# sjy-dv/coltt

Hardware: AMD Instinct MI355X
Metric: queries/sec @ recall@10, 10Mx768 HNSW (higher is better)
Workload: dtype f32

## Files before the change

### coltt_amd/_lib.py

```python
import ctypes as C
import os
import re

HERE = os.path.dirname(os.path.abspath(__file__))
COSINE, EUCLIDEAN = 0, 1
Q_NONE, Q_F16, Q_F8, Q_BF16 = 0, 1, 2, 3
SELECT_REFERENCE, SELECT_NEAREST = 0, 1
MODE_EXACT, MODE_MFMA = 0, 1
NBR_NONE = 0xFFFFFFFF

_lib = None
_env_seen = None
_KNOBS = ("COLTT_FLAT_ONE", "COLTT_FLAT_IDS_CHUNK", "COLTT_STAGING", "COLTT_EV8", "COLTT_ROWS8", "COLTT_F8_MFMA", "COLTT_VISG", "COLTT_WALK2", "COLTT_WALK2_LDS", "COLTT_BLOOM_KB",
          "COLTT_WAVES_PER_CU", "COLTT_ROWS_NT", "COLTT_ROWS_NT_MIN_MB", "COLTT_ROW_FILTER", "COLTT_ROW_FILTER_BITS", "COLTT_ROW_FILTER_UPPER", "COLTT_DESCENT_NT", "COLTT_ROW_SHADOW", "COLTT_ROW_SHADOW_BITS", "COLTT_VIS16", "COLTT_VIS16_BUCKET_BITS", "COLTT_PQ_WAVES", "COLTT_PQ_NBR", "COLTT_PQ_NBR_PATCH", "COLTT_LAT_SEQ", "COLTT_LAT_HELPERS", "COLTT_LAT_MAX_NQ", "COLTT_MW_MAX_NQ", "COLTT_VISG_BUDGET_MB")


class ColttError(RuntimeError):
    def __init__(self, code, msg):
        super().__init__(f"coltt_gpu error {code}: {msg}")
        self.code = code


def lib_path():
    return os.environ.get("COLTT_LIB", os.path.join(HERE, "libcoltt_gpu.so"))


def declared_symbols():
    hdr = open(os.path.join(HERE, "..", "include", "coltt_gpu.h")).read()
    return sorted(set(re.findall(r"\b(coltt_[a-z0-9_]+)\s*\(", hdr)))


def _sync_policy():
    global _env_seen
    get = os.environ.get
    now = tuple(get(k) for k in _KNOBS)
    if now != _env_seen:
        if _env_seen is not None:
            _lib.coltt_policy_reload()
        _env_seen = now


def lib():
    global _lib
    if _lib is not None:
        _sync_policy()
        return _lib
    if _lib is None:
        try:
            import torch
        except Exception:
            pass
        p = lib_path()
        if not os.path.exists(p):
            raise ColttError(-5, f"{p} is missing — build it with `python -m coltt_amd.build` "
                                 "(hipcc --offload-arch=gfx950); there is no CPU fallback")
        L = C.CDLL(p)
        L.coltt_last_error.restype = C.c_char_p
        L.coltt_version.restype = C.c_char_p
        if hasattr(L, "coltt_hnsw_pq_search_filtered_batch"):
            L.coltt_hnsw_pq_search_filtered_batch.restype = C.c_int
            L.coltt_hnsw_pq_search_filtered_batch.argtypes = [C.c_uint64, C.c_void_p, C.c_void_p, C.c_size_t, C.c_uint32, C.c_uint32, C.c_uint32, C.c_int,
                                                              C.c_void_p, C.c_void_p, C.c_void_p, C.c_void_p, C.c_void_p]
        if hasattr(L, "coltt_flat_mfma_eligible_host"):
            L.coltt_flat_mfma_eligible_host.restype = C.c_int
            L.coltt_flat_mfma_eligible_host.argtypes = [C.c_int, C.c_int, C.c_uint32, C.c_float, C.c_float, C.c_int]
        _lib = L
        _sync_policy()
    return _lib


def check(rc):
    if rc != 0:
        raise ColttError(rc, lib().coltt_last_error().decode("utf-8", "replace"))


def vp(a):
    if a is None:
        return C.c_void_p(0)
    if isinstance(a, int):
        return C.c_void_p(a)
    return a.ctypes.data_as(C.c_void_p)
```

### coltt_amd/csrc/common.hip

```cpp
#include "common.hpp"

#include <algorithm>
#include <cstdlib>

namespace coltt {

thread_local std::string g_last_error;
static int g_device = -1;
static std::mutex g_dev_mu;

Registry& Registry::get() {
  static Registry r;
  return r;
}
coltt_handle_t Registry::add(std::shared_ptr<Object> o) {
  std::lock_guard<std::mutex> g(mu_);
  coltt_handle_t h = next_++;
  map_[h] = std::move(o);
  return h;
}
std::shared_ptr<Object> Registry::find(coltt_handle_t h) {
  std::lock_guard<std::mutex> g(mu_);
  auto it = map_.find(h);
  return it == map_.end() ? nullptr : it->second;
}
bool Registry::erase(coltt_handle_t h) {
  std::shared_ptr<Object> keep;
  {
    std::lock_guard<std::mutex> g(mu_);
    auto it = map_.find(h);
    if (it == map_.end()) return false;
    keep = it->second;
    map_.erase(it);
  }
  WriteLock g2(keep->rw);
  return true;
}

int ensure_device() {
  int dev;
  {
    std::lock_guard<std::mutex> g(g_dev_mu);
    if (g_device < 0) {
      int n = 0;
      hipError_t e = hipGetDeviceCount(&n);
      if (e != hipSuccess || n <= 0)
        return fail(COLTT_E_DEVICE, "libcoltt_gpu: no HIP device visible (%s) — this library has no CPU fallback",
                    e == hipSuccess ? "device count 0" : hipGetErrorString(e));
      g_device = 0;
    }
    dev = g_device;
  }
  COLTT_HIP(hipSetDevice(dev));
  return COLTT_OK;
}

int default_device() { std::lock_guard<std::mutex> g(g_dev_mu); return g_device < 0 ? 0 : g_device; }

int use_device(int device) {
  COLTT_HIP(hipSetDevice(device));
  return COLTT_OK;
}

namespace {
std::shared_mutex g_pol_mu;
Policy g_policy;
bool g_policy_loaded = false;
Policy read_policy_from_env() {
  Policy p;
  auto off = [](const char* n) { const char* e = getenv(n); return e && *e == '0'; };
  auto num = [](const char* n, bool& set) -> long long { const char* e = getenv(n); set = e && *e; return set ? atoll(e) : 0; };
  bool set = false; long long v;
  p.flat_one = !off("COLTT_FLAT_ONE"); p.staging = !off("COLTT_STAGING"); p.ev8 = !off("COLTT_EV8"); { const char* e = getenv("COLTT_ROWS8"); p.rows8 = (!e || !*e) ? 1 : (*e == '0' ? 0 : (*e == '2' ? 2 : 1)); } p.f8_mfma = !off("COLTT_F8_MFMA");
  v = num("COLTT_FLAT_IDS_CHUNK", set); p.flat_ids_chunk = set && v > 0 ? (uint32_t)((std::min<long long>(v, 1ll << 30) + 31) / 32 * 32) : 0u;
  v = num("COLTT_VISG", set); p.visg = set ? (int)v : -1;
  { const char* e = getenv("COLTT_WALK2"); p.walk2 = (!e || !*e) ? 7 : (!strcmp(e, "off") ? -1 : (atoi(e) & 15)); }
  { const char* e = getenv("COLTT_WALK2_LDS"); if (!e || !*e) p.walk2_lds = 4; else if (!strcmp(e, "off")) p.walk2_lds = -1; else { const int w = atoi(e) & 6; p.walk2_lds = w ? w : -1; } }
  v = num("COLTT_BLOOM_KB", set); p.bloom_kb = set ? (int)std::max<long long>(1, std::min<long long>(64, v)) : 0;
  v = num("COLTT_WAVES_PER_CU", set); p.waves_per_cu = set ? (int)std::max<long long>(1, std::min<long long>(12, v)) : 0;
  v = num("COLTT_ROWS_NT", set); p.rows_nt = set ? (v > 0 ? 1 : (v < 0 ? -1 : 0)) : -1;
  v = num("COLTT_ROW_FILTER", set); p.row_filter = set ? (v > 0 ? 1 : 0) : -1;
  v = num("COLTT_ROW_FILTER_UPPER", set); p.row_filter_upper = set ? (v > 0 ? 1 : 0) : -1;
  v = num("COLTT_DESCENT_NT", set); p.descent_nt = set ? (v > 0 ? 1 : 0) : -1;
  p.row_shadow = !off("COLTT_ROW_SHADOW");
  v = num("COLTT_ROW_FILTER_BITS", set); p.row_filter_bits = set && (v == 8 || v == 16) ? (int)v : 0;
  { const char* e = getenv("COLTT_ROW_FILTER_BITS"); if (e && !strcmp(e, "8i")) p.row_filter_bits = 80; }
  { const char* e = getenv("COLTT_ROW_SHADOW_BITS"); p.row_shadow_bits = (!e || !*e) ? 8 : (!strcmp(e, "both") ? 24 : (atoi(e) == 16 ? 16 : 8)); }
  v = num("COLTT_ROWS_NT_MIN_MB", set); p.rows_nt_min_mb = set ? std::max<long long>(0, v) : 12288;
  p.vis16 = !off("COLTT_VIS16");
  v = num("COLTT_VIS16_BUCKET_BITS", set); p.vis16_bucket_bits = set ? (int)std::max<long long>(1, std::min<long long>(10, v)) : 0;
  v = num("COLTT_PQ_WAVES", set); p.pq_waves = set ? (int)std::max<long long>(1, std::min<long long>(16, v)) : 0;
  p.pq_nbr = !off("COLTT_PQ_NBR");
  p.pq_nbr_patch = !off("COLTT_PQ_NBR_PATCH");
  { const char* e = getenv("COLTT_LAT_SEQ"); p.lat_seq = e && *e == '1'; }
  v = num("COLTT_LAT_HELPERS", set); p.lat_helpers = set ? (int)std::max<long long>(0, std::min<long long>(3, v)) : 0;
  v = num("COLTT_LAT_MAX_NQ", set); if (!set) v = num("COLTT_MW_MAX_NQ", set);
  p.lat_knob_set = set; p.lat_max_nq = set ? (uint32_t)std::max<long long>(0, v) : 0;
  v = num("COLTT_VISG_BUDGET_MB", set); p.visg_budget_mb = set ? v : -1;
  return p;
}
}

Policy policy() {
  {
    std::shared_lock<std::shared_mutex> g(g_pol_mu);
    if (g_policy_loaded) return g_policy;
  }
  std::unique_lock<std::shared_mutex> g(g_pol_mu);
  if (!g_policy_loaded) { g_policy = read_policy_from_env(); g_policy_loaded = true; }
  return g_policy;
}

size_t max_search_ctx() {
  static const size_t v = [] { const char* e = getenv("COLTT_MAX_SEARCH_CTX"); long n = e && *e ? atol(e) : 32; return (size_t)(n < 1 ? 1 : (n > 256 ? 256 : n)); }();
  return v;
}

}

using namespace coltt;

extern "C" {

int coltt_init(int device) {
  int n = 0;
  hipError_t e = hipGetDeviceCount(&n);
  if (e != hipSuccess || n <= 0)
    return fail(COLTT_E_DEVICE, "coltt_init: no HIP device visible (%s) — this library has no CPU fallback",
                e == hipSuccess ? "device count 0" : hipGetErrorString(e));
  if (device < 0 || device >= n) return fail(COLTT_E_INVALID, "coltt_init: device %d out of range [0,%d)", device, n);
  {
    std::lock_guard<std::mutex> g(g_dev_mu);
    g_device = device;
  }
  COLTT_HIP(hipSetDevice(device));
  return COLTT_OK;
}

int coltt_device_count(void) {
  int n = 0;
  if (hipGetDeviceCount(&n) != hipSuccess) return 0;
  return n;
}

const char* coltt_last_error(void) { return g_last_error.c_str(); }

int coltt_policy_reload(void) {
  Policy p = read_policy_from_env();
  std::unique_lock<std::shared_mutex> g(g_pol_mu);
  g_policy = p; g_policy_loaded = true;
  return COLTT_OK;
}
const char* coltt_version(void) {
  return "coltt_gpu 0.6 (gfx950)";
}

}

#include "exact.hpp"
extern "C" uint64_t coltt_shard_vertex_host(uint64_t id, uint64_t shard_count) {
  return shard_count ? coltt::dev::shard_vertex(id, shard_count) : 0;
}
```

### coltt_amd/csrc/common.hpp

```cpp
#pragma once
#include <hip/hip_runtime.h>

#include <cstdarg>
#include <cstdint>
#include <cstdio>
#include <cstring>
#include <memory>
#include <condition_variable>
#include <mutex>
#include <shared_mutex>
#include <string>
#include <unordered_map>
#include <vector>

#include "../../include/coltt_gpu.h"

namespace coltt {

extern thread_local std::string g_last_error;

inline int fail(int code, const char* fmt, ...) {
  char buf[512];
  va_list ap;
  va_start(ap, fmt);
// ... 7 lines not shown
  do {                                                                                           \
    hipError_t _e = (expr);                                                                      \
    if (_e != hipSuccess)                                                                        \
      return ::coltt::fail(_e == hipErrorOutOfMemory ? COLTT_E_NOMEM : COLTT_E_DEVICE, "%s: %s", \
                           #expr, hipGetErrorString(_e));                                        \
  } while (0)

#define COLTT_TRY(expr)        \
  do {                         \
    int _rc = (expr);          \
    if (_rc != COLTT_OK) return _rc; \
  } while (0)

struct DevBuf {
  void* p = nullptr;
  size_t cap = 0;
  DevBuf() = default;
  DevBuf(const DevBuf&) = delete;
  DevBuf& operator=(const DevBuf&) = delete;
  ~DevBuf() { if (p) (void)hipFree(p); }
  int reserve(size_t bytes, bool keep = false, hipStream_t s = nullptr) {
    if (bytes <= cap) return COLTT_OK;
    size_t ncap = keep ? std::max(bytes, cap + cap / 2) : bytes;
    void* np = nullptr;
    COLTT_HIP(hipMalloc(&np, ncap));
    if (keep && p && cap) {
      hipError_t e = hipMemcpyAsync(np, p, cap, hipMemcpyDeviceToDevice, s);
      if (e == hipSuccess) e = hipStreamSynchronize(s);
      if (e != hipSuccess) {
        (void)hipFree(np);
        return ::coltt::fail(COLTT_E_DEVICE, "DevBuf::reserve copy: %s", hipGetErrorString(e));
      }
    }
    if (p) (void)hipFree(p);
    p = np;
    cap = ncap;
    return COLTT_OK;
  }
  template <class T> T* as() const { return (T*)p; }
};

struct PinnedBuf {
  void* p = nullptr;
  size_t cap = 0;
  PinnedBuf() = default;
  PinnedBuf(const PinnedBuf&) = delete;
  PinnedBuf& operator=(const PinnedBuf&) = delete;
  ~PinnedBuf() { if (p) (void)hipHostFree(p); }
  int reserve(size_t bytes) {
    if (bytes <= cap) return COLTT_OK;
    if (p) { (void)hipHostFree(p); p = nullptr; cap = 0; }
    COLTT_HIP(hipHostMalloc(&p, bytes, hipHostMallocDefault));
    cap = bytes;
    return COLTT_OK;
  }
  template <class T> T* as() const { return (T*)p; }
};
constexpr size_t SMALL_CALL_BYTES = 64 * 1024;

struct Policy {
  bool flat_one = true;
  uint32_t flat_ids_chunk = 0;
  bool staging = true;
  bool ev8 = true;
  bool f8_mfma = true;
  int rows8 = 1;
  int visg = -1;
  int walk2 = 7;
  int walk2_lds = 4;
  int bloom_kb = 0;
  int waves_per_cu = 0;
  int rows_nt = -1;
  int row_filter = -1;
  bool row_shadow = true;
  int row_filter_bits = 0;
  int row_shadow_bits = 8;
  long long rows_nt_min_mb = 12288;
  int row_filter_upper = -1;
  int descent_nt = -1;
  bool vis16 = true;
  int vis16_bucket_bits = 0;
  int pq_waves = 0;
  bool pq_nbr = true;
  bool pq_nbr_patch = true;
  bool lat_seq = false;
  int lat_helpers = 0;
  bool lat_knob_set = false;
  uint32_t lat_max_nq = 0;
  long long visg_budget_mb = -1;
};
Policy policy();
inline bool small_call_staging() { return policy().staging; }

struct Object {
  std::shared_mutex rw;
  int device = 0;
  virtual ~Object() {}
};
typedef std::shared_lock<std::shared_mutex> ReadLock;
typedef std::unique_lock<std::shared_mutex> WriteLock;

size_t max_search_ctx();
template <class C> class CtxPool {
 public:
  C* acquire() {
    std::unique_lock<std::mutex> lk(mu_);
    for (;;) {
      if (!idle_.empty()) { C* c = idle_.back(); idle_.pop_back(); return c; }
      if (all_.size() < max_search_ctx()) {
        auto c = std::make_unique<C>();
        if (c->init() != COLTT_OK) return nullptr;
        C* p = c.get(); all_.push_back(std::move(c)); return p;
      }
      cv_.wait(lk);
    }
  }
  void release(C* c) { { std::lock_guard<std::mutex> lk(mu_); idle_.push_back(c); } cv_.notify_one(); }
  size_t created() { std::lock_guard<std::mutex> lk(mu_); return all_.size(); }
 private:
  std::mutex mu_; std::condition_variable cv_;
  std::vector<std::unique_ptr<C>> all_; std::vector<C*> idle_;
};
template <class C> struct CtxLease {
  CtxPool<C>& pool; C* c;
  explicit CtxLease(CtxPool<C>& p) : pool(p), c(p.acquire()) {}
  ~CtxLease() { if (c) pool.release(c); }
  CtxLease(const CtxLease&) = delete; CtxLease& operator=(const CtxLease&) = delete;
};

class Registry {
 public:
  static Registry& get();
  coltt_handle_t add(std::shared_ptr<Object> o);
  std::shared_ptr<Object> find(coltt_handle_t h);
  bool erase(coltt_handle_t h);

 private:
  std::mutex mu_;
  std::unordered_map<coltt_handle_t, std::shared_ptr<Object>> map_;
  coltt_handle_t next_ = 0x1000;
};

template <class T> std::shared_ptr<T> lookup(coltt_handle_t h) {
  return std::dynamic_pointer_cast<T>(Registry::get().find(h));
}

int ensure_device();
int default_device();
int use_device(int device);

class DeviceScope {
 public:
  DeviceScope() = default;
  DeviceScope(const DeviceScope&) = delete;
  DeviceScope& operator=(const DeviceScope&) = delete;
  ~DeviceScope() { if (prev_ >= 0 && prev_ != cur_) (void)hipSetDevice(prev_); }
  int enter(int device) {
    if (hipGetDevice(&prev_) != hipSuccess) prev_ = -1;
    if (device < 0) { COLTT_TRY(ensure_device()); cur_ = default_device(); return COLTT_OK; }
    COLTT_TRY(use_device(device));
    cur_ = device;
    return COLTT_OK;
  }
  int device() const { return cur_; }
 private:
  int prev_ = -1, cur_ = -1;
// ... 25 lines not shown
```

### coltt_amd/csrc/hnsw.hip

```cpp
#include <algorithm>
#include <atomic>
#include <cmath>
#include <map>

#include "common.hpp"
#include "hnsw_index.hpp"
#include "exact.hpp"
#include "hnsw_dev.hpp"
#include "hnsw_walk2.hpp"
#include "hnsw_lat.hpp"
#include "hnsw_pq.hpp"
#include "prep.hpp"
#include "rows8_ingest.hpp"

#include "hnsw_kernels.hpp"
#include "filter_expr.hpp"
#include "attr_filter.hpp"
#include "hnsw_compact.hpp"

using namespace coltt;
using namespace coltt::dev;
using namespace coltt::kern;
using namespace coltt::hnsw;

// ... 878 lines not shown
  const uint64_t t = (uint64_t)blockIdx.x * blockDim.x + threadIdx.x;
  const uint64_t i = t / per;
  uint32_t n = cap;
  if (count) { const uint32_t c = *count; n = c < cap ? c : cap; }
  if (i >= n) return;
  const uint32_t slot = slots[i];
  if (slot >= n_slots) return;
  const uint32_t r = (uint32_t)(t - i * per);
  const uint32_t p = r / pieces, pc = r - p * pieces;
  const uint64_t e = (uint64_t)slot * W + p;
  const uint32_t nb = adj0[e];
  u32x4v v = {0u, 0u, 0u, 0u};
  if (nb < n_slots) v = *reinterpret_cast<const u32x4v*>(codes + (size_t)nb * row_bytes + (size_t)pc * 16);
  *reinterpret_cast<u32x4v*>(nbr + e * row_bytes + (size_t)pc * 16) = v;
}
constexpr uint64_t PQ_PATCH_MAX_LIST = 1ull << 20;
struct PqNbrPatch { bool on = false; uint32_t* d_dirty = nullptr; uint32_t cap = 0; };
PqNbrPatch pq_nbr_patch_begin(Hnsw* x, uint64_t max_listed) {
  PqNbrPatch t;
  const bool current = !x->pq_nbr_stale.load() && x->pq_nbr_ok;
  x->pq_nbr_stale.store(true);
  if (!current || !x->pq_on || max_listed > PQ_PATCH_MAX_LIST) return t;
  const Policy pol = policy();
  if (!pol.pq_nbr || !pol.pq_nbr_patch) return t;
  if (max_listed) {
    if (x->pq_dirty.reserve((2 + max_listed) * 4) != COLTT_OK) { (void)hipGetLastError(); return t; }
    if (hipMemsetAsync(x->pq_dirty.p, 0, 8, x->stream) != hipSuccess) { (void)hipGetLastError(); return t; }
    t.d_dirty = x->pq_dirty.as<uint32_t>(); t.cap = (uint32_t)max_listed;
  }
  t.on = true;
  return t;
}
int pq_nbr_patch_end(Hnsw* x, const PqNbrPatch& t, uint64_t first_new, uint64_t n_new, const uint32_t* d_slots, uint32_t n_slots_listed) {
  if (!t.on) return COLTT_OK;
  const uint32_t W = (uint32_t)x->cfg.m_max0, pieces = x->pq_row >> 4;
  if (x->pq_nbr.cap < (size_t)std::max<uint64_t>(x->cap, x->n) * W * x->pq_row || x->pq_done < x->n) return COLTT_OK;
  const uint32_t* adj0 = x->adj0.as<uint32_t>(); const uint8_t* codes = x->pq_codes.as<uint8_t>(); uint8_t* nbr = x->pq_nbr.as<uint8_t>();
  if (n_new) {
    const uint64_t total = n_new * W * pieces, e0 = first_new * W;
    pq_nbr_build_kernel<<<(unsigned)ceil_div(total, 256), 256, 0, x->stream>>>(adj0 + e0, codes, nbr + e0 * x->pq_row, total, x->pq_row);
  }
  const uint32_t* list = t.d_dirty ? t.d_dirty + 2 : d_slots;
  const uint32_t lcap = t.d_dirty ? t.cap : n_slots_listed;
  if (lcap) pq_nbr_patch_kernel<<<(unsigned)ceil_div((uint64_t)lcap * W * pieces, 256), 256, 0, x->stream>>>(adj0, codes, nbr, list, t.d_dirty, lcap, W, x->pq_row, (uint32_t)x->n);
  COLTT_HIP(hipGetLastError());
  uint32_t listed = n_slots_listed;
  if (t.d_dirty) COLTT_HIP(hipMemcpyAsync(&listed, t.d_dirty, 4, hipMemcpyDeviceToHost, x->stream));
  COLTT_HIP(hipStreamSynchronize(x->stream));
  if (listed > lcap) return COLTT_OK;
  x->pq_nbr_patches.fetch_add(1); x->pq_nbr_patched_rows.fetch_add(n_new + listed);
  x->pq_nbr_stale.store(false);
  return COLTT_OK;
}
constexpr size_t PQ_WAVES_CAP = 12;
bool pq_geom(Hnsw* x, uint32_t ef, bool force_hbm, PqGeom& out, uint32_t filt_cap = 0) {
  PqGeom s{};
  s.ef = ef; s.ef_pad = (ef + 63) & ~63u;
  const size_t fixed = (size_t)s.ef_pad * 8 + ((size_t)pq_walk_table_rows(x->pq_row >> 4) << pq_lut_shift(x)) * 2
                     + (filt_cap ? (size_t)((filt_cap + 63u) & ~63u) * 8 : 0);
  if (fixed > 160 * 1024) return false;
  const bool hbm_ok = x->vis_stride != 0 && x->vis_regions > 0;
  uint32_t hcap = std::min<uint32_t>(32768u, std::max<uint32_t>(8192u, next_pow2(ef * 48u)));
  const bool lds_fits = fixed + (size_t)hcap * 4 <= 160 * 1024;
  if (!force_hbm && !(wants_visg(policy(), ef) && hbm_ok) && lds_fits) { s.variant = 0; s.vis_words = hcap; s.lds = fixed + (size_t)hcap * 4; }
  else {
    if (!hbm_ok) return false;
    s.variant = 2; s.vis_words = 0; s.lds = fixed;
  }
  {
    const Policy pol = policy();
    const size_t cap = pol.pq_waves > 0 ? (size_t)pol.pq_waves : PQ_WAVES_CAP;
    s.per_cu = (uint32_t)std::max<size_t>(1, std::min<size_t>(cap, (160 * 1024) / s.lds));
  }
  out = s;
  return true;
}

}

namespace coltt {
namespace hnsw {
int launch_pq_walk(Hnsw* x, HCtx* c, const PqGeom& sg, bool nbr, uint32_t grid, uint32_t region_base, const unsigned short* lut, uint32_t nq, uint32_t k,
                   uint32_t rerank, uint32_t* counter, uint32_t* surv, uint32_t* surv_cnt, unsigned long long* stats, const FilterView* fv, uint32_t fcap,
                   const PqFiltQuery* pd) {
  const uint32_t sh = pq_lut_shift(x);
  const uint32_t np = x->pq_row >> 4;
  typedef void (*pq_kern_t)(GraphView, int32_t, int32_t, const unsigned short*, const uint8_t*, const uint8_t*, uint32_t, uint32_t, uint32_t, uint32_t, uint32_t, uint32_t, uint32_t, uint32_t,
                            uint32_t*, uint32_t*, uint32_t*, unsigned long long*, uint8_t*, size_t, uint32_t*, FilterView, uint32_t);
  pq_kern_t kern;
#define COLTT_PQKF(LS, NP, F, P) (sg.variant == 0 ? (pq_kern_t)hnsw_pq_search_kernel<0, VIS_LDS, LS, NP, false, F, P> : nbr ? (pq_kern_t)hnsw_pq_search_kernel<2, VIS_HBM, LS, NP, true, F, P> : (pq_kern_t)hnsw_pq_search_kernel<2, VIS_HBM, LS, NP, false, F, P>)
#define COLTT_PQK(LS, NP) (pd ? COLTT_PQKF(LS, NP, true, true) : fv ? COLTT_PQKF(LS, NP, true, false) : COLTT_PQKF(LS, NP, false, false))
  if (sh == 5 && np == 4) kern = COLTT_PQK(5, 4);
  else if (sh == 4 && np == 4) kern = COLTT_PQK(4, 4);
  else if (sh == 8 && np == 2) kern = COLTT_PQK(8, 2);
  else if (sh == 8 && np == 6) kern = COLTT_PQK(8, 6);
  else if (sh == 4) kern = COLTT_PQK(4, 0);
  else if (sh == 5) kern = COLTT_PQK(5, 0);
  else if (sh == 8) kern = COLTT_PQK(8, 0);
  else kern = COLTT_PQK(0, 0);
#undef COLTT_PQK
#undef COLTT_PQKF
  COLTT_HIP(hipFuncSetAttribute(reinterpret_cast<const void*>(kern), hipFuncAttributeMaxDynamicSharedMemorySize, (int)sg.lds));
  kern<<<grid, 64, sg.lds, c->stream>>>(x->view(), x->entry, x->entry_level, lut, x->pq_codes.as<uint8_t>(), nbr ? x->pq_nbr.as<uint8_t>() : nullptr, x->pq_row, sh, nq, k, sg.ef, sg.ef_pad, rerank,
                                        sg.vis_words, counter, surv, surv_cnt, stats, x->w_visg.as<uint8_t>() + (size_t)region_base * x->vis_stride,
                                        (size_t)x->vis_stride, x->w_vepoch.as<uint32_t>() + region_base,
                                        pd ? FilterView{reinterpret_cast<const uint32_t*>(pd), 0u} : fv ? *fv : FilterView{nullptr, 0u}, fcap);
  COLTT_HIP(hipGetLastError());
  return COLTT_OK;
}
}
}

namespace {
}

namespace coltt {
namespace kern {
__global__ __launch_bounds__(64) void hnsw_pq_select_kernel(const unsigned long long* __restrict__ keys, const uint32_t* __restrict__ surv_cnt, uint32_t ef_pad, uint32_t k,
                                                            const uint64_t* __restrict__ ids, uint64_t* __restrict__ out_ids, float* __restrict__ out_scores,
                                                            uint32_t* __restrict__ out_counts, const PqFiltQuery* __restrict__ pd = nullptr) {
  extern __shared__ __attribute__((aligned(16))) uint8_t smem[];
  unsigned long long* const res = reinterpret_cast<unsigned long long*>(smem);
  const uint32_t qi = blockIdx.x, r = surv_cnt[qi];
  const uint32_t row = pd ? pd[qi].row : qi;
  const int lane_in = threadIdx.x;
  for (uint32_t i = (uint32_t)lane_in; i < r; i += 64) res[i] = keys[(size_t)qi * ef_pad + i];
  wave_sync();
  const uint32_t n = r < k ? r : k;
  for (uint32_t t = 0; t < n; t++) {
    const int lane = opaque_lane(lane_in);
    unsigned long long best = ~0ull; uint32_t bi = 0;
    for (uint32_t i = (uint32_t)lane; i < r; i += 64) { const unsigned long long e = res[i]; if (e < best) { best = e; bi = i; } }
    const unsigned long long km = wave_min_u64(best);
    if (best == km && km != ~0ull) {
      const uint32_t slot = (uint32_t)km >> 1;
      out_ids[(size_t)row * k + t] = ids ? ids[slot] : (uint64_t)slot;
      out_scores[(size_t)row * k + t] = __uint_as_float((uint32_t)(km >> 32));
      res[bi] = ~0ull;
    }
    wave_sync();
  }
  if (lane_in == 0) out_counts[row] = n;
}
}
}

namespace {
template <int METRIC, int QUANT>
int launch_pq_rerank_for(Hnsw* x, HCtx* c, const PqGeom& sg, uint32_t q0, uint32_t nq, uint32_t k, const uint32_t* surv, const uint32_t* surv_cnt,
                     unsigned long long* keys, uint64_t* oi, float* os, uint32_t* oc, const PqFiltQuery* pd = nullptr, const float* pd_qe = nullptr,
                     const float* pd_qn = nullptr) {
  const dim3 grid(ceil_div(sg.ef_pad, 32), nq);
  const GraphView g = x->view();
  const float* qe = c->w_qeff.as<float>() + (size_t)q0 * x->dim; const float* qn = c->w_qn.as<float>() + q0;
  if (pd) { qe = pd_qe; qn = pd_qn; q0 = 0; }
  if (x->r8) hnsw_pq_rerank_kernel<METRIC, QUANT, true><<<grid, 64, 0, c->stream>>>(g, qe, qn, surv, surv_cnt, sg.ef_pad, keys);
  else hnsw_pq_rerank_kernel<METRIC, QUANT, false><<<grid, 64, 0, c->stream>>>(g, qe, qn, surv, surv_cnt, sg.ef_pad, keys);
  const size_t lds = (size_t)sg.ef_pad * 8;
  COLTT_HIP(hipFuncSetAttribute(reinterpret_cast<const void*>(hnsw_pq_select_kernel), hipFuncAttributeMaxDynamicSharedMemorySize, (int)lds));
  hnsw_pq_select_kernel<<<nq, 64, lds, c->stream>>>(keys, surv_cnt, sg.ef_pad, k, g.ids, oi + (size_t)q0 * k, os + (size_t)q0 * k, oc + q0, pd);
  COLTT_HIP(hipGetLastError());
  return COLTT_OK;
}
}

namespace coltt {
namespace hnsw {
int launch_pq_rerank(Hnsw* x, HCtx* c, const PqGeom& sg, uint32_t q0, uint32_t nq, uint32_t k, const uint32_t* surv, const uint32_t* surv_cnt,
                     unsigned long long* keys, uint64_t* oi, float* os, uint32_t* oc, const PqFiltQuery* pd, const float* pd_qe, const float* pd_qn) {
  int rc;
#define COLTT_LP_ARGS x, c, sg, q0, nq, k, surv, surv_cnt, keys, oi, os, oc, pd, pd_qe, pd_qn
#define COLTT_LP(Q) rc = x->metric == COLTT_COSINE ? launch_pq_rerank_for<M_COS, Q>(COLTT_LP_ARGS) : launch_pq_rerank_for<M_L2, Q>(COLTT_LP_ARGS)
  if (x->quant == COLTT_Q_NONE) { COLTT_LP(Q_NONE); } else { COLTT_LP(Q_F16); }
#undef COLTT_LP
#undef COLTT_LP_ARGS
  return rc;
}

int pq_walk_geom(Hnsw* x, uint32_t ef, bool force_hbm, uint32_t fcap, PqGeom& sg) {
  const Policy pol = policy();
  if (wants_visg(pol, ef) || force_hbm) COLTT_TRY(ensure_visg(x, pol));
  bool have = pq_geom(x, ef, force_hbm, sg, fcap);
  if (!have && !force_hbm) { COLTT_TRY(ensure_visg(x, pol)); have = pq_geom(x, ef, true, sg, fcap); }
  if (!have) return fail(COLTT_E_UNSUPPORTED, "hnsw_pq_search: dim %u / ef %u / %u sub-vectors need more than the CU's 160 KiB of LDS", x->dim, ef, x->pq_shape.m);
  return COLTT_OK;
}
}
}

namespace {

int pq_search_once(Hnsw* x, HCtx* c, const float* queries, bool on_device, size_t nq, uint32_t k, uint32_t ef_override, uint32_t rerank,
                   uint64_t* out_ids, float* out_scores, uint32_t* out_counts, coltt_hnsw_stats* stats, uint64_t* out_n_exact, bool force_hbm, bool* retry_hbm,
                   const FilterView* fv = nullptr) {
  *retry_hbm = false;
  if (stats) std::memset(stats, 0, sizeof(*stats));
  if (out_n_exact) *out_n_exact = 0;
  if (nq == 0) return COLTT_OK;
  if (k == 0) return fail(COLTT_E_INVALID, "hnsw_pq_search: k must be >= 1");
  if (!x->pq_on) return fail(COLTT_E_INVALID, "hnsw_pq_search: the index carries no product-quantiser codes (coltt_hnsw_pq_attach)");
  if (x->pq_done != x->n) return fail(COLTT_E_DEVICE, "hnsw_pq_search: codes cover %llu of %llu slots", (unsigned long long)x->pq_done, (unsigned long long)x->n);
  uint64_t* d_oi = out_ids; float* d_os = out_scores; uint32_t* d_oc = out_counts;
  if (!on_device) {
    COLTT_TRY(c->w_out_ids.reserve(nq * k * 8)); COLTT_TRY(c->w_out_sc.reserve(nq * k * 4)); COLTT_TRY(c->w_out_cnt.reserve(nq * 4));
    d_oi = c->w_out_ids.as<uint64_t>(); d_os = c->w_out_sc.as<float>(); d_oc = c->w_out_cnt.as<uint32_t>();
  }
  if (x->entry < 0) {
    COLTT_HIP(hipMemsetAsync(d_oc, 0, nq * 4, c->stream));
    if (!on_device) COLTT_HIP(hipMemcpyAsync(out_counts, d_oc, nq * 4, hipMemcpyDeviceToHost, c->stream));
    COLTT_HIP(hipStreamSynchronize(c->stream));
    return COLTT_OK;
  }
  const uint32_t ef = std::max<uint32_t>(ef_override ? ef_override : (uint32_t)x->cfg.ef, k);
  if (ef > 4096) return fail(COLTT_E_UNSUPPORTED, "hnsw_pq_search: ef=%u > 4096", ef);
  PqGeom sg;
  const uint32_t fcap = fv ? pq_filt_cap(ef, k, rerank) : 0u;
  COLTT_TRY(pq_walk_geom(x, ef, force_hbm, fcap, sg));
  uint32_t grid = (uint32_t)std::min<size_t>(nq, (size_t)256 * sg.per_cu);
  RegionLease lease;
  if (sg.variant != 0) { acquire_regions(x, grid, lease); grid = lease.count; }
  const float* d_q = queries;
  if (!on_device) {
    COLTT_TRY(c->w_qraw.reserve(nq * x->dim * 4));
    COLTT_HIP(hipMemcpyAsync(c->w_qraw.p, queries, nq * x->dim * 4, hipMemcpyHostToDevice, c->stream));
    d_q = c->w_qraw.as<float>();
  }
  COLTT_TRY(prep_queries_any(x, c, d_q, nq));
  bool nbr = false;
  if (sg.variant != 0) COLTT_TRY(ensure_pq_nbr(x, c->stream, &nbr));
  const uint32_t lsh = pq_lut_shift(x);
  const size_t lut_q = ((size_t)x->pq_row << lsh) * 2;
  const size_t group = std::max<size_t>(1, std::min<size_t>({nq, (256ull << 20) / lut_q, (256ull << 20) / ((size_t)sg.ef_pad * 12), (size_t)32768}));
  COLTT_TRY(c->w_pack.reserve(group * lut_q + group * 4));
  COLTT_TRY(c->w_surv.reserve(group * sg.ef_pad * 4)); COLTT_TRY(c->w_scnt.reserve(group * 4)); COLTT_TRY(c->w_keys.reserve(group * sg.ef_pad * 8));
  COLTT_TRY(c->w_misc.reserve(256));
  uint8_t* misc = c->w_misc.as<uint8_t>();
  uint32_t* counter = reinterpret_cast<uint32_t*>(misc);
  unsigned long long* d_stats = reinterpret_cast<unsigned long long*>(misc + 16);
  COLTT_HIP(hipMemsetAsync(misc, 0, 256, c->stream));
  COLTT_HIP(hipEventRecord(c->ev0, c->stream));
  for (size_t q0 = 0; q0 < nq; q0 += group) {
    const size_t gn = std::min(group, nq - q0);
    COLTT_TRY(pq_lut16_batch(c->stream, x->pq_cb.as<float>(), x->pq_shape, c->w_qeff.as<float>() + q0 * x->dim, gn, x->pq_row, lsh,
                             reinterpret_cast<uint32_t*>(c->w_pack.as<uint8_t>() + group * lut_q), c->w_pack.as<unsigned short>()));
    if (q0) COLTT_HIP(hipMemsetAsync(counter, 0, 4, c->stream));
    COLTT_TRY(launch_pq_walk(x, c, sg, nbr, (uint32_t)std::min<size_t>(grid, gn), lease.base, c->w_pack.as<unsigned short>(), (uint32_t)gn, k, rerank, counter, c->w_surv.as<uint32_t>(),
                             c->w_scnt.as<uint32_t>(), d_stats, fv, fcap));
    COLTT_TRY(launch_pq_rerank(x, c, sg, (uint32_t)q0, (uint32_t)gn, k, c->w_surv.as<uint32_t>(), c->w_scnt.as<uint32_t>(), c->w_keys.as<unsigned long long>(), d_oi, d_os, d_oc));
  }
  COLTT_HIP(hipEventRecord(c->ev1, c->stream));
  if (x->dense && x->dense_base) add_base_kernel<<<ceil_div(nq * k, 256), 256, 0, c->stream>>>(d_oi, nq * k, x->dense_base);
  unsigned long long h_stats[5] = {0, 0, 0, 0, 0};
  if (!on_device) {
    COLTT_HIP(hipMemcpyAsync(out_ids, d_oi, nq * k * 8, hipMemcpyDeviceToHost, c->stream));
    COLTT_HIP(hipMemcpyAsync(out_scores, d_os, nq * k * 4, hipMemcpyDeviceToHost, c->stream));
    COLTT_HIP(hipMemcpyAsync(out_counts, d_oc, nq * 4, hipMemcpyDeviceToHost, c->stream));
  }
  COLTT_HIP(hipMemcpyAsync(h_stats, d_stats, 40, hipMemcpyDeviceToHost, c->stream));
#ifdef COLTT_PHASE_TIMING
  unsigned long long h_pt[8] = {0};
  COLTT_HIP(hipMemcpyAsync(h_pt, d_stats + 8, 64, hipMemcpyDeviceToHost, c->stream));
#endif
  COLTT_HIP(hipStreamSynchronize(c->stream));
#ifdef COLTT_PHASE_TIMING
  {
    static const char* nm[8] = {"pop", "adjacency", "visited", "codes+table sum", "admission/evict/flush", "prologue(table, upper levels)", "flush+re-rank+writeout", "-"};
    double tot = 0; for (int i = 0; i < 7; i++) tot += (double)h_pt[i];
    fprintf(stderr, "[phase pq] nq=%zu ef=%u variant=%d per_cu=%u:", nq, sg.ef, sg.variant, sg.per_cu);
    for (int i = 0; i < 7; i++) fprintf(stderr, " %s %.1f%%", nm[i], 100.0 * (double)h_pt[i] / tot);
    fprintf(stderr, "  | ticks/query %.0f, per expansion %.0f\n", tot / (double)nq, tot / (double)std::max<unsigned long long>(1, h_stats[1]));
  }
#endif
  float ms = 0.f;
  (void)hipEventElapsedTime(&ms, c->ev0, c->ev1);
  x->last_ms.store(ms);
  if (sg.variant == 0 && (h_stats[4] & 8ull)) { *retry_hbm = true; return COLTT_OK; }
  if (h_stats[4]) return fail(COLTT_E_DEVICE, "hnsw_pq_search: traversal watchdog tripped (code %llu)", h_stats[4]);
  if (stats) { stats->n_dist = h_stats[0]; stats->n_exp = h_stats[1]; stats->n_hops = h_stats[2]; stats->n_visit_resets = 0; }
  if (out_n_exact) *out_n_exact = h_stats[3];
  return COLTT_OK;
}
int pq_search_common(Hnsw* x, HCtx* c, const float* queries, bool on_device, size_t nq, uint32_t k, uint32_t ef_override, uint32_t rerank,
                     uint64_t* out_ids, float* out_scores, uint32_t* out_counts, coltt_hnsw_stats* stats, uint64_t* out_n_exact) {
  bool retry = false;
  COLTT_TRY(pq_search_once(x, c, queries, on_device, nq, k, ef_override, rerank, out_ids, out_scores, out_counts, stats, out_n_exact, false, &retry));
  if (retry) COLTT_TRY(pq_search_once(x, c, queries, on_device, nq, k, ef_override, rerank, out_ids, out_scores, out_counts, stats, out_n_exact, true, &retry));
  return COLTT_OK;
}
}

namespace coltt {
namespace hnsw {
int pq_search_filtered_walk(Hnsw* x, HCtx* c, const FilterView& fv, const float* queries, size_t nq, uint32_t k, uint32_t ef_walk, uint32_t rerank,
                            uint64_t* out_ids, float* out_scores, uint32_t* out_counts, coltt_hnsw_stats* stats, uint64_t* out_n_exact) {
  bool retry = false;
  COLTT_TRY(pq_search_once(x, c, queries, false, nq, k, ef_walk, rerank, out_ids, out_scores, out_counts, stats, out_n_exact, false, &retry, &fv));
  if (retry) COLTT_TRY(pq_search_once(x, c, queries, false, nq, k, ef_walk, rerank, out_ids, out_scores, out_counts, stats, out_n_exact, true, &retry, &fv));
  return COLTT_OK;
}
}
}

namespace {

__global__ void hnsw_unlink_kernel(GraphView g, const uint32_t* __restrict__ nbs, const int32_t* __restrict__ lvl, uint32_t n) {
  uint32_t t = blockIdx.x * blockDim.x + threadIdx.x;
  if (t >= n) return;
  uint32_t W;
  uint32_t* row = const_cast<uint32_t*>(adj_row(g, nbs[t], lvl[t], W));
  float* drow = lvl[t] == 0 ? g.adj0_d + (size_t)nbs[t] * g.mMax0 : g.adjU_d + ((size_t)g.upper_off[nbs[t]] + (uint32_t)(lvl[t] - 1)) * g.mMax;
  float* nrow = (lvl[t] == 0 && g.adj0_n) ? g.adj0_n + (size_t)nbs[t] * g.mMax0 : nullptr;
  float2* mrow = (lvl[t] == 0 && g.adj0_m) ? g.adj0_m + (size_t)nbs[t] * g.mMax0 : nullptr;
  uint32_t m = 0;
  for (uint32_t i = 0; i < W && row[i] != NBR_NONE; i++) {
    uint32_t sl = row[i]; float dd = drow[i];
    if (!is_deleted(g, sl)) { row[m] = sl; drow[m] = dd; if (nrow) nrow[m] = nrow[i]; if (mrow) mrow[m] = mrow[i]; m++; }
  }
  for (; m < W; m++) { row[m] = NBR_NONE; drow[m] = 0.f; if (nrow) nrow[m] = 0.f; if (mrow) mrow[m] = float2{0.f, 0.f}; }
}

int hnsw_undense(Hnsw* x) {
  if (!x->dense) return COLTT_OK;
  x->h_ids.resize(x->n);
  x->id2slot.reserve(x->n * 2);
  for (uint64_t s = 0; s < x->n; s++) {
    x->h_ids[s] = x->dense_base + s;
    if (!(x->h_del.size() > (s >> 5) && ((x->h_del[s >> 5] >> (s & 31)) & 1u))) x->id2slot[x->dense_base + s] = (uint32_t)s;
  }
  x->dense = false;
  COLTT_TRY(x->ids.reserve(std::max<uint64_t>(x->cap, 1024) * 8, false, x->stream));
// ... 1034 lines not shown
int coltt_hnsw_pq_info(coltt_handle_t h, uint32_t* out_m, uint32_t* out_c, int32_t* out_metric, uint64_t* out_coded) {
  auto x = lookup<Hnsw>(h);
  if (!x) return fail(COLTT_E_NOT_FOUND, "hnsw_pq_info: unknown handle");
  ReadLock g(x->rw);
  if (out_m) *out_m = x->pq_on ? x->pq_shape.m : 0;
  if (out_c) *out_c = x->pq_on ? x->pq_shape.C : 0;
  if (out_metric) *out_metric = x->pq_on ? x->pq_shape.metric : -1;
  if (out_coded) *out_coded = x->pq_on ? x->pq_done : 0;
  return COLTT_OK;
}

int coltt_hnsw_pq_fetch_codes(coltt_handle_t h, uint64_t first_slot, uint64_t n, uint8_t* out_codes) {
  auto x = lookup<Hnsw>(h);
  if (!x) return fail(COLTT_E_NOT_FOUND, "hnsw_pq_fetch_codes: unknown handle");
  ReadLock g(x->rw);
  COLTT_DEVICE(x->device);
  if (!x->pq_on) return fail(COLTT_E_INVALID, "hnsw_pq_fetch_codes: no quantiser attached");
  if (first_slot + n > x->pq_done) return fail(COLTT_E_INVALID, "hnsw_pq_fetch_codes: slots [%llu,%llu) outside the %llu coded ones", (unsigned long long)first_slot, (unsigned long long)(first_slot + n), (unsigned long long)x->pq_done);
  if (n == 0) return COLTT_OK;
  if (!out_codes) return fail(COLTT_E_INVALID, "hnsw_pq_fetch_codes: NULL out");
  COLTT_HIP(hipMemcpy2D(out_codes, x->pq_shape.m, x->pq_codes.as<uint8_t>() + first_slot * x->pq_row, x->pq_row, x->pq_shape.m, n, hipMemcpyDeviceToHost));
  return COLTT_OK;
}

namespace {
int pq_nbr_state(const Hnsw* x) {
  if (!policy().pq_nbr || !x->pq_on) return 0;
  if (x->pq_nbr_stale.load()) return x->pq_nbr_built ? 2 : 0;
  return x->pq_nbr_ok ? 1 : 0;
}
}

int coltt_hnsw_pq_nbr_stats(coltt_handle_t h, uint64_t* out_builds, uint64_t* out_patches, uint64_t* out_patched_rows, int32_t* out_state) {
  auto x = lookup<Hnsw>(h);
  if (!x) return fail(COLTT_E_NOT_FOUND, "hnsw_pq_nbr_stats: unknown handle");
  ReadLock g(x->rw);
  std::lock_guard<std::mutex> gn(x->pq_nbr_mu);
  if (out_builds) *out_builds = x->pq_nbr_builds.load();
  if (out_patches) *out_patches = x->pq_nbr_patches.load();
  if (out_patched_rows) *out_patched_rows = x->pq_nbr_patched_rows.load();
  if (out_state) *out_state = pq_nbr_state(x.get());
  return COLTT_OK;
}

int coltt_hnsw_pq_fetch_nbr(coltt_handle_t h, uint64_t first_slot, uint64_t n, uint8_t* out_blocks) {
  auto x = lookup<Hnsw>(h);
  if (!x) return fail(COLTT_E_NOT_FOUND, "hnsw_pq_fetch_nbr: unknown handle");
  ReadLock g(x->rw);
  COLTT_DEVICE(x->device);
  std::lock_guard<std::mutex> gn(x->pq_nbr_mu);
  const int st = pq_nbr_state(x.get());
  if (st != 1) return fail(COLTT_E_UNSUPPORTED, "hnsw_pq_fetch_nbr: the neighbourhood blocks are %s", st == 2 ? "stale (the next product-quantised walk above ef 128 rebuilds them)" : "not kept");
  if (first_slot > x->n || n > x->n - first_slot) return fail(COLTT_E_INVALID, "hnsw_pq_fetch_nbr: slots [%llu,%llu) outside [0,%llu)", (unsigned long long)first_slot, (unsigned long long)(first_slot + n), (unsigned long long)x->n);
  if (n == 0) return COLTT_OK;
  if (!out_blocks) return fail(COLTT_E_INVALID, "hnsw_pq_fetch_nbr: NULL out");
  const size_t blk = (size_t)x->cfg.m_max0 * x->pq_row;
  COLTT_HIP(hipMemcpy(out_blocks, x->pq_nbr.as<uint8_t>() + first_slot * blk, n * blk, hipMemcpyDeviceToHost));
  return COLTT_OK;
}

int coltt_hnsw_pq_search(coltt_handle_t h, const float* queries, size_t nq, uint32_t k, uint32_t ef_override, uint32_t rerank,
                         uint64_t* out_ids, float* out_scores, uint32_t* out_counts, coltt_hnsw_stats* stats, uint64_t* out_n_exact) {
  auto x = lookup<Hnsw>(h);
  if (!x) return fail(COLTT_E_NOT_FOUND, "hnsw_pq_search: unknown handle");
  if (nq && (!queries || !out_ids || !out_scores || !out_counts)) return fail(COLTT_E_INVALID, "hnsw_pq_search: NULL buffer");
  ReadLock g(x->rw);
  COLTT_DEVICE(x->device);
  CtxLease<HCtx> ctx(x->pool);
  if (!ctx.c) return COLTT_E_DEVICE;
  return pq_search_common(x.get(), ctx.c, queries, false, nq, k, ef_override, rerank, out_ids, out_scores, out_counts, stats, out_n_exact);
}
int coltt_hnsw_pq_search_device(coltt_handle_t h, const float* d_queries, size_t nq, uint32_t k, uint32_t ef_override, uint32_t rerank,
                                uint64_t* d_out_ids, float* d_out_scores, uint32_t* d_out_counts, coltt_hnsw_stats* stats, uint64_t* out_n_exact) {
  auto x = lookup<Hnsw>(h);
  if (!x) return fail(COLTT_E_NOT_FOUND, "hnsw_pq_search_device: unknown handle");
  if (nq && (!d_queries || !d_out_ids || !d_out_scores || !d_out_counts)) return fail(COLTT_E_INVALID, "hnsw_pq_search_device: NULL buffer");
  ReadLock g(x->rw);
  COLTT_DEVICE(x->device);
  CtxLease<HCtx> ctx(x->pool);
  if (!ctx.c) return COLTT_E_DEVICE;
  return pq_search_common(x.get(), ctx.c, d_queries, true, nq, k, ef_override, rerank, d_out_ids, d_out_scores, d_out_counts, stats, out_n_exact);
}

int coltt_hnsw_rows8_searches(coltt_handle_t h, uint64_t* out_launches, int32_t* out_has_copy) {
  auto x = lookup<Hnsw>(h);
  if (!x) return fail(COLTT_E_NOT_FOUND, "hnsw_rows8_searches: unknown handle");
  ReadLock g(x->rw);
  if (out_launches) *out_launches = x->ev8_launches.load();
  if (out_has_copy) *out_has_copy = x->r8 ? 1 : 0;
  return COLTT_OK;
}

int coltt_hnsw_visited_stats(coltt_handle_t h, int32_t* out_kind, uint32_t* out_waves_per_cu, uint32_t* out_grid, uint64_t* out_launches16, uint64_t* out_stash_max, uint64_t* out_visited_max) {
  auto x = lookup<Hnsw>(h);
  if (!x) return fail(COLTT_E_NOT_FOUND, "hnsw_visited_stats: unknown handle");
  ReadLock g(x->rw);
  if (out_kind) *out_kind = x->last_vis_kind.load();
  if (out_waves_per_cu) *out_waves_per_cu = x->last_per_cu.load();
  if (out_grid) *out_grid = x->last_grid.load();
  if (out_launches16) *out_launches16 = x->v16_launches.load();
  if (out_stash_max) *out_stash_max = x->last_stash_max.load();
  if (out_visited_max) *out_visited_max = x->last_visited_max.load();
  return COLTT_OK;
}

int coltt_hnsw_search_plan_host(const coltt_hnsw_plan_facts* facts, size_t nq, uint32_t k, uint32_t ef_override, int force, coltt_hnsw_search_plan* out) {
  if (!facts || !out) return fail(COLTT_E_INVALID, "hnsw_search_plan_host: NULL facts or out");
  if (nq == 0 || ef_override == 0) return fail(COLTT_E_INVALID, "hnsw_search_plan_host: nq and ef_override must be >= 1 (the index's default ef is not among the facts)");
  SearchPlan sp;
  const int rc = plan_search(*facts, policy(), nq, k, ef_override, force, sp);
  *out = rc == COLTT_OK ? sp : SearchPlan{};
  return rc;
}

int coltt_hnsw_search_plan_facts(coltt_handle_t h, coltt_hnsw_plan_facts* out_facts) {
  auto x = lookup<Hnsw>(h);
  if (!x) return fail(COLTT_E_NOT_FOUND, "hnsw_search_plan_facts: unknown handle");
  if (!out_facts) return fail(COLTT_E_INVALID, "hnsw_search_plan_facts: NULL out");
  ReadLock g(x->rw);
  *out_facts = plan_facts(x.get());
  return COLTT_OK;
}

int coltt_last_kernel_ms(coltt_handle_t h, float* out_ms) {
  if (!out_ms) return fail(COLTT_E_INVALID, "last_kernel_ms: NULL out");
  if (auto x = lookup<Hnsw>(h)) { *out_ms = x->last_ms.load(); return COLTT_OK; }
  return coltt_last_kernel_ms_flat(h, out_ms);
}

}

namespace {

struct HnswAttr : Object {
  coltt_handle_t index = 0; uint64_t gen = 0;
  int type = COLTT_ATTR_I64;
  uint32_t slots = 0;
  uint64_t cap = 0, n_set = 0;
  DevBuf vals;
  DevBuf set;
  std::vector<uint32_t> h_set;
  ~HnswAttr() override { (void)hipSetDevice(device); }
};

inline bool live_slot_of(const Hnsw* x, uint64_t id, uint32_t& s) {
  if (x->dense) {
    if (id < x->dense_base || id - x->dense_base >= x->n) return false;
    s = (uint32_t)(id - x->dense_base);
    return !(x->h_del.size() > (s >> 5) && ((x->h_del[s >> 5] >> (s & 31)) & 1u));
  }
  auto it = x->id2slot.find(id);
  if (it == x->id2slot.end()) return false;
  s = it->second;
  return true;
}


int filter_eval_common(coltt_handle_t h, const char* who, const int32_t* progs, const uint64_t* prog_off, size_t n_out,
                       const coltt_handle_t* leaves, size_t n_leaves, const coltt_attr_pred* preds, size_t n_preds,
                       uint64_t* out_allowed, coltt_handle_t* out) {
  auto x = lookup<Hnsw>(h);
  if (!x) return fail(COLTT_E_NOT_FOUND, "%s: unknown index handle", who);
  if (n_out == 0) return COLTT_OK;
  if (!out) return fail(COLTT_E_INVALID, "%s: out is NULL", who);
  if (!prog_off) return fail(COLTT_E_INVALID, "%s: NULL programme offsets", who);
  if (n_leaves && !leaves) return fail(COLTT_E_INVALID, "%s: NULL leaves", who);
// ... 398 lines not shown
```

### coltt_amd/csrc/hnsw_index.hpp

```cpp
#pragma once
#include <algorithm>
#include <atomic>

#include "common.hpp"
#include "hnsw_dev.hpp"

namespace coltt {
namespace hnsw {
using namespace coltt::dev;

struct HCtx {
  hipStream_t stream = nullptr;
  hipEvent_t ev0 = nullptr, ev1 = nullptr;
  DevBuf w_qraw, w_qeff, w_qn, w_out_ids, w_out_sc, w_out_cnt, w_misc, w_pack;
  DevBuf w_surv, w_scnt, w_keys;
  DevBuf w_mbox;
  DevBuf w_fdesc;
  PinnedBuf h_in, h_out;
  const void* occ_kern = nullptr; size_t occ_lds = 0; int occ_per_cu = 0;
  int init() {
    COLTT_HIP(hipStreamCreateWithFlags(&stream, hipStreamNonBlocking));
    COLTT_HIP(hipEventCreate(&ev0));
    COLTT_HIP(hipEventCreate(&ev1));
    return COLTT_OK;
  }
  ~HCtx() {
    if (ev0) (void)hipEventDestroy(ev0);
    if (ev1) (void)hipEventDestroy(ev1);
    if (stream) (void)hipStreamDestroy(stream);
  }
};

struct Hnsw : Object {
  uint32_t dim = 0; int metric = 0, quant = 0; size_t stride = 0;
  coltt_hnsw_cfg cfg{};
  uint64_t n = 0 , live = 0, cap = 0, n_upper = 0, ucap = 0;
  int32_t entry = -1, entry_level = 0;
  bool any_deleted = false;
  DevBuf rows, norms, ids, adj0, adj0_d, adj0_n, upper_off, adjU, adjU_d, del_bits;
  bool r8 = false;
  DevBuf w_stage;
  std::atomic<uint64_t> ev8_launches{0};
  bool shadow = false;
  DevBuf rows_h;
  bool shadow8 = false;
  DevBuf rows_b, rows_m, adj0_m;
  void drop_shadow8() {
    shadow8 = false;
    for (DevBuf* b : {&rows_b, &rows_m, &adj0_m}) if (b->p) { (void)hipFree(b->p); b->p = nullptr; b->cap = 0; }
    (void)hipGetLastError();
  }
  bool has_shadow8() const { return shadow8 && rows_b.p && rows_m.p && adj0_m.p; }
  bool has_shadow16() const { return shadow && rows_h.p; }
  std::atomic<uint64_t> flt_up_launches{0}, flt_up_shadow_rows{0}, flt_up_rejected{0}, flt_up_f32_rows{0};
  std::atomic<uint64_t> flt_launches{0}, flt_rejected{0}, flt_f32_rows{0}, flt_shadow_rows{0};
  std::atomic<int32_t> last_vis_kind{-1}; std::atomic<uint32_t> last_per_cu{0}, last_grid{0};
  std::atomic<uint64_t> v16_launches{0}, last_stash_max{0}, last_visited_max{0};
  void drop_shadow() { shadow = false; if (rows_h.p) { (void)hipFree(rows_h.p); rows_h.p = nullptr; rows_h.cap = 0; } (void)hipGetLastError(); }
  bool pq_on = false; PqShape pq_shape; uint32_t pq_row = 0 ; uint64_t pq_done = 0;
  DevBuf pq_cb, pq_codes, pq_stage;
  DevBuf pq_nbr; bool pq_nbr_ok = false; std::atomic<bool> pq_nbr_stale{true}; std::mutex pq_nbr_mu;
  bool pq_nbr_built = false;
  DevBuf pq_dirty;
  std::atomic<uint64_t> pq_nbr_builds{0}, pq_nbr_patches{0}, pq_nbr_patched_rows{0};
  bool dense = true; uint64_t dense_base = 0;
  std::unordered_map<uint64_t, uint32_t> id2slot;
  std::vector<uint64_t> h_ids;
  std::vector<int32_t> h_levels;
  std::vector<uint32_t> h_upper_off;
  std::vector<uint32_t> h_del;
  hipStream_t stream = nullptr;
  std::atomic<float> last_ms{0.f};
  CtxPool<HCtx> pool;
  DevBuf w_raw, w_misc;
  DevBuf b_head, b_req, b_levels; uint64_t head_cap = 0;
  DevBuf w_visg, w_vepoch; uint64_t vis_stride = 0; uint32_t vis_regions = 0, vis_want = 0;
  std::mutex vis_mu; std::condition_variable vis_cv; std::vector<uint8_t> vis_busy;
  coltt_hnsw_stats build_stats{};
  uint64_t gen = 0;
  ~Hnsw() override {
    (void)hipSetDevice(device);
    if (stream) (void)hipStreamDestroy(stream);
  }
  GraphView view() const {
    GraphView g;
    g.rows = rows.as<uint8_t>(); g.stride = stride; g.norms = norms.as<float>();
    g.rows8 = r8 ? rows.as<uint8_t>() : nullptr;
    g.ids = dense ? nullptr : ids.as<uint64_t>();
    g.adj0 = adj0.as<uint32_t>(); g.adj0_d = adj0_d.as<float>(); g.upper_off = upper_off.as<uint32_t>();
    g.adj0_n = metric == COLTT_COSINE ? adj0_n.as<float>() : nullptr;
    g.adjU = adjU.as<uint32_t>(); g.adjU_d = adjU_d.as<float>();
    g.del_bits = any_deleted ? del_bits.as<uint32_t>() : nullptr;
    g.mMax = (uint32_t)cfg.m_max; g.mMax0 = (uint32_t)cfg.m_max0; g.dim = (int)dim;
    g.rows_h = shadow ? rows_h.as<uint8_t>() : nullptr;
    g.rows_b = shadow8 ? rows_b.as<uint8_t>() : nullptr;
    g.rows_m = shadow8 ? rows_m.as<float2>() : nullptr;
    g.adj0_m = shadow8 ? adj0_m.as<float2>() : nullptr;
    return g;
  }
  int reserve(uint64_t slots, uint64_t upper_rows) {
    if (slots > cap) {
      uint64_t nc = std::max<uint64_t>({slots, cap + cap / 2, 1024});
      COLTT_TRY(rows.reserve(nc * stride, true, stream));
      if (shadow && rows_h.reserve(nc * (size_t)dim * 2, true, stream) != COLTT_OK) drop_shadow();
      if (shadow8 && (rows_b.reserve(nc * (size_t)dim, true, stream) != COLTT_OK || rows_m.reserve(nc * 8, true, stream) != COLTT_OK ||
                      adj0_m.reserve(nc * cfg.m_max0 * 8, true, stream) != COLTT_OK)) drop_shadow8();
      COLTT_TRY(norms.reserve(nc * 4, true, stream));
      if (!dense) COLTT_TRY(ids.reserve(nc * 8, true, stream));
      COLTT_TRY(adj0.reserve(nc * cfg.m_max0 * 4, true, stream));
      COLTT_TRY(adj0_d.reserve(nc * cfg.m_max0 * 4, true, stream));
      if (metric == COLTT_COSINE) COLTT_TRY(adj0_n.reserve(nc * cfg.m_max0 * 4, true, stream));
      COLTT_TRY(upper_off.reserve(nc * 4, true, stream));
      size_t old_words = (cap + 31) / 32, new_words = (nc + 31) / 32;
      COLTT_TRY(del_bits.reserve(new_words * 4, true, stream));
      if (new_words > old_words) COLTT_HIP(hipMemsetAsync(del_bits.as<uint32_t>() + old_words, 0, (new_words - old_words) * 4, stream));
      cap = nc;
    }
    if (upper_rows > ucap) {
      uint64_t nc = std::max<uint64_t>({upper_rows, ucap + ucap / 2, 256});
      COLTT_TRY(adjU.reserve(nc * cfg.m_max * 4, true, stream));
      COLTT_TRY(adjU_d.reserve(nc * cfg.m_max * 4, true, stream));
      ucap = nc;
    }
    return COLTT_OK;
  }
};

typedef coltt_hnsw_plan_facts PlanFacts;
typedef coltt_hnsw_search_plan SearchPlan;

struct SearchGeom { uint32_t ef, ef_pad, hcap; size_t lds; bool visg; uint32_t max_grid; };

struct RegionLease {
  Hnsw* x = nullptr; uint32_t base = 0, count = 0;
  ~RegionLease() {
    if (!x || !count) return;
    { std::lock_guard<std::mutex> g(x->vis_mu); for (uint32_t i = 0; i < count; i++) x->vis_busy[base + i] = 0; }
    x->vis_cv.notify_all();
  }
};

struct PqGeom { uint32_t ef, ef_pad, vis_words; size_t lds; int variant;  uint32_t per_cu; };

struct FilterSlab {
  int device = 0;
  DevBuf bits, lists;
  ~FilterSlab() { (void)hipSetDevice(device); }
};

struct HnswFilter : Object {
  coltt_handle_t index = 0; uint64_t gen = 0;
  uint32_t slots = 0;
  uint64_t allowed = 0;
  DevBuf bits;
  DevBuf list;
  std::shared_ptr<FilterSlab> slab;
  ~HnswFilter() override {
    (void)hipSetDevice(device);
    if (slab) { bits.p = nullptr; list.p = nullptr; }
  }
};

inline uint32_t pq_lut_shift(const Hnsw* x) { uint32_t sh = 4; while ((1u << sh) < x->pq_shape.C) sh++; return sh; }
inline uint32_t pq_filt_cap(uint32_t ef, uint32_t k, uint32_t rerank) { return rerank == 0 ? ef : std::min(std::max(rerank, k), ef); }

int prep_queries_any(Hnsw* x, HCtx* c, const float* d_qraw, size_t nq, uint32_t* zero64 = nullptr);
void add_base(hipStream_t stream, uint64_t* ids, size_t n, uint64_t base);
int ensure_visg(Hnsw* x, const Policy& pol);
void acquire_regions(Hnsw* x, uint32_t want, RegionLease& out);
PlanFacts plan_facts(const Hnsw* x);
bool wants_visg(const Policy& pol, uint32_t ef);
SearchGeom walk_geom(const PlanFacts& f, const Policy& pol, uint32_t ef, uint32_t allowed = 0);
uint32_t resident_waves(const Policy& pol, int quant, size_t lds, int w2 = -1, bool vis16 = false);
inline bool walk2_shipped(bool hbm, int w2) { return hbm ? (w2 == 6 || w2 == 7) : w2 == 4; }
int plan_search(const PlanFacts& f, const Policy& pol, size_t nq, uint32_t k, uint32_t ef, int force, SearchPlan& out);
int ensure_pq_nbr(Hnsw* x, hipStream_t stream, bool* use);
int pq_walk_geom(Hnsw* x, uint32_t ef, bool force_hbm, uint32_t fcap, PqGeom& sg);
int launch_pq_walk(Hnsw* x, HCtx* c, const PqGeom& sg, bool nbr, uint32_t grid, uint32_t region_base, const unsigned short* lut, uint32_t nq, uint32_t k,
                   uint32_t rerank, uint32_t* counter, uint32_t* surv, uint32_t* surv_cnt, unsigned long long* stats, const FilterView* fv = nullptr, uint32_t fcap = 0,
                   const PqFiltQuery* pd = nullptr);
int launch_pq_rerank(Hnsw* x, HCtx* c, const PqGeom& sg, uint32_t q0, uint32_t nq, uint32_t k, const uint32_t* surv, const uint32_t* surv_cnt,
                     unsigned long long* keys, uint64_t* oi, float* os, uint32_t* oc, const PqFiltQuery* pd = nullptr, const float* pd_qe = nullptr,
                     const float* pd_qn = nullptr);
int pq_search_filtered_walk(Hnsw* x, HCtx* c, const FilterView& fv, const float* queries, size_t nq, uint32_t k, uint32_t ef_walk, uint32_t rerank,
                            uint64_t* out_ids, float* out_scores, uint32_t* out_counts, coltt_hnsw_stats* stats, uint64_t* out_n_exact);

int launch_search2(Hnsw* x, HCtx* c, const SearchPlan& sp, uint32_t grid, uint32_t region_base, uint32_t nq, uint32_t k, uint32_t* counter,
                   uint64_t* oi, float* os, uint32_t* oc, unsigned long long* stats);

}
}
```

### coltt_amd/csrc/hnsw_kernels.hpp

```cpp
#pragma once
#include "common.hpp"
#include "exact.hpp"
#include "hnsw_dev.hpp"
#include "hnsw_walk2.hpp"
#include "hnsw_lat.hpp"
#include "hnsw_pq.hpp"

namespace coltt {
namespace kern {
using namespace coltt::dev;

template <int METRIC, int QUANT, bool VISG, bool R8, bool FILTER, bool PERQ = false>
__device__ __forceinline__ void search_one_wave(uint8_t* smem, GraphView g, int32_t entry, int32_t entry_level,
                                                const float* __restrict__ q_eff, const float* __restrict__ qnorms,
                                                uint32_t nq, uint32_t k, uint32_t ef, uint32_t ef_pad, uint32_t hcap,
                                                uint32_t* __restrict__ counter, uint64_t* __restrict__ out_ids,
                                                float* __restrict__ out_scores, uint32_t* __restrict__ out_counts,
                                                unsigned long long* __restrict__ stats, uint8_t* __restrict__ visg,
                                                size_t vis_stride, uint32_t* __restrict__ vis_epoch, FilterView fv,
                                                const FiltQuery* __restrict__ fq = nullptr) {
  constexpr int PROF = VISG ? PROF_SEARCH_HBM : PROF_SEARCH_LDS;
  const int lane = threadIdx.x;
  WaveCtx w;
  size_t off = ((size_t)g.dim * 4 + 15) & ~(size_t)15;
// ... 370 lines not shown
  size_t off = (lat_q_floats(g.dim) * 4 + 15) & ~(size_t)15;
  w.qs = reinterpret_cast<float*>(smem);
  w.res0 = reinterpret_cast<unsigned long long*>(smem + off);
  LatShared* xs = reinterpret_cast<LatShared*>(w.res0 + (size_t)ef_pad);
  uint8_t* stage = reinterpret_cast<uint8_t*>(xs + 1);
  w.vis = reinterpret_cast<uint32_t*>(stage + (TP == LAT_TP_STAGED ? (size_t)LAT_ROWS * (g.stride + LAT_PAD) : (size_t)0));
  w.ef_pad = ef_pad; w.hcap = hcap; w.hcap_mask = hcap - 1;
  w.visg = nullptr; w.vis_bytes = 0; w.epoch = 0; w.bloom = nullptr; w.bloom_words = 0; w.bloom_shift = 0;
  for (;;) {
    __syncthreads();
    if (threadIdx.x == 0) xs->ctl[1] = atomicAdd(counter, 1u);
    __syncthreads();
    const uint32_t qi = xs->ctl[1];
    if (qi >= nq) break;
    w.n_dist = w.n_exp = w.n_hops = w.n_resets = 0; w.err = 0;
#ifdef COLTT_PHASE_TIMING
    for (int i_ = 0; i_ < 8; i_++) w.pt[i_] = 0;
    w.t_last = __builtin_amdgcn_s_memtime();
#endif
    {
      const int n8 = g.dim >> 3, n8p = lat_n8p(g.dim);
      for (int e = threadIdx.x; e < g.dim; e += 256) {
        const float v = q_eff[(size_t)qi * g.dim + e];
        if (e < n8 * 8) w.qs[(size_t)(e & 7) * n8p + (e >> 3)] = v; else w.qs[(size_t)8 * n8p + (e - n8 * 8)] = v;
      }
    }
    w.qnorm = qnorms[qi];
    if (threadIdx.x < LAT_ROWS) { xs->nb[threadIdx.x] = threadIdx.x == 0 ? (uint32_t)entry : NBR_NONE; xs->fresh[threadIdx.x] = threadIdx.x == 0 ? 1u : 0u; }
    lat_chunk<METRIC, QUANT, TP>(g, w, xs, stage, wave, lane);
    uint32_t cur = (uint32_t)entry;
    float curd = xs->d[0];
    w.n_dist += 1;
    __syncthreads();
    for (int l = entry_level; l > 0; l--) greedy_level_lat<METRIC, QUANT, TP>(g, w, xs, stage, cur, curd, l, wave, lane);
#ifdef COLTT_PHASE_TIMING
    if (wave == 0) { unsigned long long t_ = __builtin_amdgcn_s_memtime(); w.pt[6] += t_ - w.t_last; w.t_last = t_; }
#endif
    w.n_dist += 1;
    uint32_t len;
    if constexpr (!SEQ) {
      search_level_lat3<METRIC, QUANT, TP>(g, w, xs, stage, cur, curd, ef, wave, lane, len, hint_box, helpers);
    } else if (wave == 0) {
      if (lane == 0) xs->ctl[0] = 1u;
      LatEval<METRIC, QUANT, TP> ev{xs, stage};
      search_level2<METRIC, QUANT, PROF_SEARCH_LDS, W2_DELTA, VIS_LDS, true>(g, w, cur, curd, ef, lane, len, ev);
      wave_sync();
      if (lane == 0) xs->ctl[0] = 0u;
      lds_barrier();
    } else {
      len = 0;
      lat_companion<METRIC, QUANT, TP>(g, w, xs, stage, wave, lane);
    }
    if (wave == 0) {
      const uint32_t n = len < k ? len : k;
      for (uint32_t i = lane; i < n; i += 64) {
        const unsigned long long e = w.res0[i];
        const uint32_t slot = (uint32_t)e >> 1;
        out_ids[(size_t)qi * k + i] = g.ids ? g.ids[slot] : (uint64_t)slot;
        out_scores[(size_t)qi * k + i] = __uint_as_float((uint32_t)(e >> 32));
      }
      if (lane == 0) {
        out_counts[qi] = n;
        atomicAdd(&stats[0], (unsigned long long)w.n_dist);
        atomicAdd(&stats[1], (unsigned long long)w.n_exp);
        atomicAdd(&stats[2], (unsigned long long)w.n_hops);
        if (w.err) atomicOr(&stats[4], (unsigned long long)w.err);
#ifdef COLTT_PHASE_TIMING
        for (int i_ = 0; i_ < 8; i_++) atomicAdd(&stats[8 + i_], w.pt[i_]);
#endif
      }
    }
  }
  if (hint_box && threadIdx.x == 0) __hip_atomic_store(hint_box + LAT_HELPERS_MAX, 1ull, __ATOMIC_RELAXED, __HIP_MEMORY_SCOPE_AGENT);
}



template <int OPT, int VISMODE, int LS, int NP = 0, bool NBR = false, bool FILTER = false, bool PERQ = false>
__global__ __launch_bounds__(64) __attribute__((amdgpu_waves_per_eu(3))) void hnsw_pq_search_kernel(GraphView g, int32_t entry, int32_t entry_level, const unsigned short* __restrict__ lut_g,
                                                            const uint8_t* __restrict__ codes, const uint8_t* __restrict__ nbrc, uint32_t row_bytes, uint32_t lut_shift, uint32_t nq, uint32_t k,
                                                            uint32_t ef, uint32_t ef_pad, uint32_t rerank, uint32_t vis_words,
                                                            uint32_t* __restrict__ counter, uint32_t* __restrict__ surv, uint32_t* __restrict__ surv_cnt,
                                                            unsigned long long* __restrict__ stats, uint8_t* __restrict__ visg,
                                                            size_t vis_stride, uint32_t* __restrict__ vis_epoch, FilterView fv, uint32_t fcap) {
  extern __shared__ __attribute__((aligned(16))) uint8_t smem[];
  const int lane = threadIdx.x;
  WaveCtx w;
  unsigned short* const lut = reinterpret_cast<unsigned short*>(smem);
  if constexpr (LS != 0) {
    if ((uint32_t)(uintptr_t)(__attribute__((address_space(3))) uint8_t*)smem != 0u) { if (lane == 0) atomicOr(&stats[4], 128ull); return; }
  }
  static_assert(!PERQ || FILTER, "a descriptor per query is the filtered batch's");
  const size_t off_table = ((size_t)pq_walk_table_rows(row_bytes >> 4) << lut_shift) * 2;
  w.qs = nullptr; w.qp = nullptr; w.scr = nullptr;
  FiltSet fs;
  (void)fs;
  if constexpr (FILTER) { fs.len = 0; fs.f = fv; }
  auto lay_out = [&](uint32_t ef_pad_q, uint32_t fcap_q, uint32_t vis_words_q) {
    size_t off = off_table;
    w.res0 = reinterpret_cast<unsigned long long*>(smem + off); off += (size_t)ef_pad_q * 8;
    w.ef_pad = ef_pad_q;
    if constexpr (FILTER) { fs.r = reinterpret_cast<unsigned long long*>(smem + off); off += (size_t)((fcap_q + 63u) & ~63u) * 8; fs.cap = fcap_q; }
    if constexpr (VISMODE == VIS_LDS) {
      w.vis = reinterpret_cast<uint32_t*>(smem + off); off += (size_t)vis_words_q * 4;
      w.hcap = vis_words_q; w.hcap_mask = vis_words_q - 1;
      w.bloom = nullptr; w.bloom_words = 0; w.bloom_shift = 0;
    } else {
      w.vis = nullptr; w.hcap = 0; w.hcap_mask = 0;
      w.bloom = reinterpret_cast<uint32_t*>(smem + off); off += (size_t)vis_words_q * 4;
      w.bloom_words = vis_words_q; w.bloom_shift = 32u - (uint32_t)__builtin_ctz(vis_words_q | 0x80000000u);
    }
  };
  if constexpr (!PERQ) lay_out(ef_pad, fcap, vis_words);
  if constexpr (VISMODE == VIS_LDS) { w.visg = nullptr; w.vis_bytes = 0; w.epoch = 0; }
  else { w.visg = visg + (size_t)blockIdx.x * vis_stride; w.vis_bytes = vis_stride; w.epoch = vis_epoch[blockIdx.x]; }
  AdcEval<LS, NP, NBR> ev; ev.codes = codes; ev.row_bytes = row_bytes; ev.lut = lut; ev.lut_shift = lut_shift; ev.nbrc = nbrc; ev.nbr_stride = g.mMax0 * row_bytes;
  ev.hsel = (uint32_t)lane & 1u;
  for (;;) {
    const uint32_t qt = atomicAdd(counter, lane == 0 ? 1u : 0u);
    const uint32_t qi = (uint32_t)__shfl((int)qt, 0, 64);
    if (qi >= nq) break;
    if constexpr (PERQ) {
      const uint32_t* dw = reinterpret_cast<const uint32_t*>(reinterpret_cast<const PqFiltQuery*>(fv.bits) + qi);
      auto rf = [&](int i) { return (uint32_t)__builtin_amdgcn_readfirstlane((int)dw[i]); };
      fs.f = FilterView{reinterpret_cast<const uint32_t*>(((uint64_t)rf(1) << 32) | rf(0)), rf(2)};
      ef = rf(3);
      lay_out(rf(4), rf(6), rf(5));
    }
    w.n_dist = w.n_exp = w.n_hops = w.n_resets = 0; w.err = 0;
#ifdef COLTT_PHASE_TIMING
    for (int i_ = 0; i_ < 8; i_++) w.pt[i_] = 0;
    w.t_last = __builtin_amdgcn_s_memtime();
#endif
    wave_sync();
    {
      const u32x4v* src = reinterpret_cast<const u32x4v*>(lut_g + ((size_t)qi * row_bytes << lut_shift));
      u32x4v* dst = reinterpret_cast<u32x4v*>(lut);
      const uint32_t psh = lut_shift - 3;
      const uint32_t total = row_bytes << psh;
      const uint32_t js = 16u * (((row_bytes >> 4) + 1u) >> 1);
      for (uint32_t i = (uint32_t)lane; i < total; i += 64) {
        const uint32_t j = i >> psh, within = i & ((1u << psh) - 1u);
        const uint32_t r = j < js ? 2u * j : 2u * (j - js) + 1u;
        dst[(r << psh) + within] = src[i];
      }
    }
    w.qnorm = 0.f;
    wave_sync();
    uint32_t cur = (uint32_t)entry;
    float curd = ev.adc(cur);
    w.n_dist += 1;
    for (int l = entry_level; l > 0; l--) greedy_level_adc(g, w, ev, cur, curd, l, lane);
    w.n_dist += 1;
    COLTT_PT(w, 5)
    uint32_t len;
    uint32_t r;
    if constexpr (FILTER) {
      search_level2<M_L2, Q_F16, PROF_SEARCH_HBM, OPT, VISMODE, true, AdcEval<LS, NP, NBR>&, true>(g, w, cur, curd, ef, lane, len, ev, &fs);
      r = fs.len;
      if constexpr (PERQ) {
        const uint32_t qerr = (uint32_t)__shfl((int)w.err, 0, 64);
        if (qerr) {
          if (lane == 0) { const_cast<PqFiltQuery*>(reinterpret_cast<const PqFiltQuery*>(fv.bits))[qi].err = qerr; surv_cnt[qi] = 0u; atomicOr(&stats[4], (unsigned long long)qerr); }
          continue;
        }
      }
      for (uint32_t i = (uint32_t)lane; i < r; i += 64) surv[(size_t)qi * ef_pad + i] = (uint32_t)fs.r[i] >> 1;
    } else {
      search_level2<M_L2, Q_F16, PROF_SEARCH_HBM, OPT, VISMODE, true>(g, w, cur, curd, ef, lane, len, ev);
      r = rerank == 0 ? len : (rerank > k ? rerank : k);
      r = r < len ? r : len;
      for (uint32_t i = (uint32_t)lane; i < r; i += 64) surv[(size_t)qi * ef_pad + i] = (uint32_t)w.res0[i] >> 1;
    }
    COLTT_PT(w, 6)
    if (lane == 0) {
#ifdef COLTT_PHASE_TIMING
      for (int i_ = 0; i_ < 8; i_++) atomicAdd(&stats[8 + i_], w.pt[i_]);
#endif
      surv_cnt[qi] = r;
      atomicAdd(&stats[0], (unsigned long long)w.n_dist);
      atomicAdd(&stats[1], (unsigned long long)w.n_exp);
      atomicAdd(&stats[2], (unsigned long long)w.n_hops);
      atomicAdd(&stats[3], (unsigned long long)r);
      if (w.err) atomicOr(&stats[4], (unsigned long long)w.err);
    }
  }
  if constexpr (VISMODE == VIS_HBM) { if (lane == 0) vis_epoch[blockIdx.x] = w.epoch; }
}

template <int METRIC, int QUANT, bool R8>
__global__ __launch_bounds__(64) void hnsw_pq_rerank_kernel(GraphView g, const float* __restrict__ q_eff, const float* __restrict__ qnorms, const uint32_t* __restrict__ surv,
                                                            const uint32_t* __restrict__ surv_cnt, uint32_t ef_pad, unsigned long long* __restrict__ keys) {
  const uint32_t qi = blockIdx.y, r = surv_cnt[qi];
  if (blockIdx.x * 32u >= r) return;
  const int lane = threadIdx.x, half = lane & 1, p = lane >> 1;
  WaveCtx w;
  w.qs = const_cast<float*>(q_eff + (size_t)qi * g.dim); w.qnorm = qnorms[qi];
  const uint32_t i = blockIdx.x * 32u + (uint32_t)p;
  const bool valid = i < r;
  const uint32_t slot = surv[(size_t)qi * ef_pad + (valid ? i : blockIdx.x * 32u)];
  const float d = eval_pair<METRIC, QUANT, PROF_SEARCH_HBM, R8>(g, w, slot, half);
  if (valid && half == 0) keys[(size_t)qi * ef_pad + i] = ((unsigned long long)__float_as_uint(d) << 32) | ((unsigned long long)slot << 1);
}

constexpr uint32_t FILT_QG = 8;
template <int METRIC, int QUANT, bool R8>
__global__ __launch_bounds__(64) void hnsw_filter_scan_kernel(GraphView g, const float* __restrict__ q_eff, const float* __restrict__ qnorms, uint32_t nq,
                                                              uint32_t qg, const uint32_t* __restrict__ slots, uint32_t n_slots, uint32_t chunk, uint32_t k,
                                                              uint32_t k_pad, unsigned long long* __restrict__ part, uint32_t* __restrict__ part_cnt,
                                                              unsigned long long* __restrict__ stats) {
  extern __shared__ __attribute__((aligned(16))) uint8_t smem[];
  const int lane_in = threadIdx.x;
  const uint32_t q0 = blockIdx.y * qg, nchunks = gridDim.x;
  const uint32_t nqg = nq - q0 < qg ? nq - q0 : qg;
  const size_t qstride = ((size_t)g.dim + 3) & ~(size_t)3;
  float* const qs = reinterpret_cast<float*>(smem);
  unsigned long long* const top = reinterpret_cast<unsigned long long*>(qs + (size_t)qg * qstride);
  for (uint32_t j = 0; j < nqg; j++)
// ... 118 lines not shown
```

### coltt_amd/csrc/hnsw_pq.hpp

```cpp
#pragma once
#include "hnsw_walk2.hpp"

namespace coltt {
namespace dev {

__host__ __device__ __forceinline__ constexpr uint32_t pq_walk_table_rows(uint32_t pieces) { return 2u * ((pieces + 1u) / 2u) * 16u; }
template <int LS = 0, int NP = 0, bool NBR = false> struct AdcEval {
  const uint8_t* codes; uint32_t row_bytes;
  const unsigned short* lut;
  uint32_t lut_shift;
  const uint8_t* nbrc; uint32_t nbr_stride;
  uint32_t hsel;
  static constexpr int NR = NP ? (NP + 1) / 2 : 4;
  static constexpr bool BIAS = LS != 0 && LS <= 7;
  __device__ __forceinline__ int pieces() const { return NP ? NP : (int)(row_bytes >> 4); }
  __device__ __forceinline__ int first_piece() const { return hsel ? (pieces() + 1) >> 1 : 0; }
  __device__ __forceinline__ int my_pieces() const { const int np = pieces(), ph = (np + 1) >> 1; return hsel ? np - ph : ph; }
  static __device__ __forceinline__ float pair_total(float part) {
    const float other = __builtin_bit_cast(float, __builtin_amdgcn_mov_dpp(__builtin_bit_cast(int, part), 0xB1, 0xf, 0xf, true));
    return part + other;
  }
  static __device__ __forceinline__ float acc(float s, uint32_t h) {
    float r; const float one = 1.0f;
    asm("v_fma_mix_f32 %0, %1, %2, %3 op_sel_hi:[1,0,0]" : "=v"(r) : "v"(h), "v"(one), "v"(s));
    return r;
  }
  template <int B> static __device__ __forceinline__ uint32_t byte2(uint32_t v) {
    uint32_t r; const uint32_t one = 1u;
    if constexpr (B == 0) asm("v_lshlrev_b32_sdwa %0, %1, %2 dst_sel:DWORD dst_unused:UNUSED_PAD src0_sel:DWORD src1_sel:BYTE_0" : "=v"(r) : "v"(one), "v"(v));
    else if constexpr (B == 1) asm("v_lshlrev_b32_sdwa %0, %1, %2 dst_sel:DWORD dst_unused:UNUSED_PAD src0_sel:DWORD src1_sel:BYTE_1" : "=v"(r) : "v"(one), "v"(v));
    else if constexpr (B == 2) asm("v_lshlrev_b32_sdwa %0, %1, %2 dst_sel:DWORD dst_unused:UNUSED_PAD src0_sel:DWORD src1_sel:BYTE_2" : "=v"(r) : "v"(one), "v"(v));
    else asm("v_lshlrev_b32_sdwa %0, %1, %2 dst_sel:DWORD dst_unused:UNUSED_PAD src0_sel:DWORD src1_sel:BYTE_3" : "=v"(r) : "v"(one), "v"(v));
    return r;
  }
  template <int B> __device__ __forceinline__ uint32_t entry(uint32_t jl, uint32_t sh, uint32_t v) const {
    return *reinterpret_cast<const unsigned short*>(reinterpret_cast<const uint8_t*>(lut) + ((size_t)(2u * jl + hsel) << (sh + 1)) + byte2<B>(v));
  }
  u32x4e raw[NR];
  static constexpr bool CHUNK_ADJ = false;
  static constexpr bool RADJ = false;
  static constexpr bool BOUNDED = true;
  static constexpr bool ROWPF = NBR;
  static constexpr bool EARLY = NBR;
  __device__ __forceinline__ uint32_t chunk_adj(int, int) const { return NBR_NONE; }
  __device__ __forceinline__ void load_from(const uint8_t* row, u32x4e (&r)[NR]) const {
    const u32x4e* p = reinterpret_cast<const u32x4e*>(row) + first_piece();
    if constexpr (NP != 0 && NP % 2 == 0) {
#pragma unroll
      for (int i = 0; i < NR; i++) r[i] = p[i];
    } else {
      const int cnt = my_pieces();
#pragma unroll
      for (int i = 0; i < NR; i++) if (i < cnt) r[i] = p[i];
    }
  }
  __device__ __forceinline__ void load(uint32_t slot, u32x4e (&r)[NR]) const { load_from(codes + (size_t)slot * row_bytes, r); }
  template <int J> static __device__ __forceinline__ float sum8(float s, uint32_t v0, uint32_t v1, uint32_t kadd) {
    static_assert(LS != 0, "sum8 needs the table's row length at compile time");
    uint32_t t0, t1, t2, t3, t4, t5, t6, t7;
    const uint32_t one = 1u; const float onef = 1.0f;
    constexpr int R = 2 << (LS + 1);
    if constexpr (!BIAS) {
      asm volatile(
        "v_lshlrev_b32_sdwa %1, %11, %9 dst_sel:DWORD dst_unused:UNUSED_PAD src0_sel:DWORD src1_sel:BYTE_0\n\t"
        "v_lshlrev_b32_sdwa %2, %11, %9 dst_sel:DWORD dst_unused:UNUSED_PAD src0_sel:DWORD src1_sel:BYTE_1\n\t"
        "v_lshlrev_b32_sdwa %3, %11, %9 dst_sel:DWORD dst_unused:UNUSED_PAD src0_sel:DWORD src1_sel:BYTE_2\n\t"
        "v_lshlrev_b32_sdwa %4, %11, %9 dst_sel:DWORD dst_unused:UNUSED_PAD src0_sel:DWORD src1_sel:BYTE_3\n\t"
        "v_lshlrev_b32_sdwa %5, %11, %10 dst_sel:DWORD dst_unused:UNUSED_PAD src0_sel:DWORD src1_sel:BYTE_0\n\t"
        "v_lshlrev_b32_sdwa %6, %11, %10 dst_sel:DWORD dst_unused:UNUSED_PAD src0_sel:DWORD src1_sel:BYTE_1\n\t"
        "v_lshlrev_b32_sdwa %7, %11, %10 dst_sel:DWORD dst_unused:UNUSED_PAD src0_sel:DWORD src1_sel:BYTE_2\n\t"
        "v_lshlrev_b32_sdwa %8, %11, %10 dst_sel:DWORD dst_unused:UNUSED_PAD src0_sel:DWORD src1_sel:BYTE_3\n\t"
        "v_add_u32 %1, %21, %1\n\t" "v_add_u32 %2, %21, %2\n\t" "v_add_u32 %3, %21, %3\n\t" "v_add_u32 %4, %21, %4\n\t"
        "v_add_u32 %5, %21, %5\n\t" "v_add_u32 %6, %21, %6\n\t" "v_add_u32 %7, %21, %7\n\t" "v_add_u32 %8, %21, %8\n\t"
        "ds_read_u16 %1, %1 offset:%13\n\t"
        "ds_read_u16 %2, %2 offset:%14\n\t"
        "ds_read_u16 %3, %3 offset:%15\n\t"
        "ds_read_u16 %4, %4 offset:%16\n\t"
        "ds_read_u16 %5, %5 offset:%17\n\t"
        "ds_read_u16 %6, %6 offset:%18\n\t"
        "ds_read_u16 %7, %7 offset:%19\n\t"
        "ds_read_u16 %8, %8 offset:%20\n\t"
        "s_waitcnt lgkmcnt(7)\n\t" "v_fma_mix_f32 %0, %1, %12, %0 op_sel_hi:[1,0,0]\n\t"
        "s_waitcnt lgkmcnt(6)\n\t" "v_fma_mix_f32 %0, %2, %12, %0 op_sel_hi:[1,0,0]\n\t"
        "s_waitcnt lgkmcnt(5)\n\t" "v_fma_mix_f32 %0, %3, %12, %0 op_sel_hi:[1,0,0]\n\t"
        "s_waitcnt lgkmcnt(4)\n\t" "v_fma_mix_f32 %0, %4, %12, %0 op_sel_hi:[1,0,0]\n\t"
        "s_waitcnt lgkmcnt(3)\n\t" "v_fma_mix_f32 %0, %5, %12, %0 op_sel_hi:[1,0,0]\n\t"
        "s_waitcnt lgkmcnt(2)\n\t" "v_fma_mix_f32 %0, %6, %12, %0 op_sel_hi:[1,0,0]\n\t"
        "s_waitcnt lgkmcnt(1)\n\t" "v_fma_mix_f32 %0, %7, %12, %0 op_sel_hi:[1,0,0]\n\t"
        "s_waitcnt lgkmcnt(0)\n\t" "v_fma_mix_f32 %0, %8, %12, %0 op_sel_hi:[1,0,0]"
// ... 123 lines not shown
```

### coltt_amd/csrc/pq.hip

```cpp
#include <algorithm>
#include <atomic>
#include <type_traits>

#include "common.hpp"
#include "exact.hpp"
#include "select.hpp"

using namespace coltt;
using namespace coltt::dev;

namespace {

typedef float f32x2 __attribute__((ext_vector_type(2)));
constexpr int PQ_LDS_MAX = 152 * 1024;

template <int KIND, int LEN = 0>
__device__ __forceinline__ float pq_dist(const float* __restrict__ x, const float* __restrict__ y, int len_rt) {
  const int len = LEN > 0 ? LEN : len_rt;
  float acc[32];
#pragma unroll
  for (int u = 0; u < 32; u++) acc[u] = 0.f;
#define PQ_BLOCK_(I_)                                                                                   \
  _Pragma("unroll") for (int u = 0; u < 32; u++) {                                                      \
    const float xv = x[(I_) + u], yv = y[(I_) + u];                                                     \
    if constexpr (KIND == 1) { const float d = xv - yv; acc[u] = __builtin_fmaf(d, d, acc[u]); }        \
    else acc[u] = __builtin_fmaf(xv, yv, acc[u]);                                                       \
  }
  int i = 0;
  if constexpr (LEN > 0) {
#pragma unroll
    for (int b = 0; b < LEN / 32; b++) { PQ_BLOCK_(b * 32) }
  } else {
    for (; len - i >= 32; i += 32) { PQ_BLOCK_(i) }
  }
#undef PQ_BLOCK_
  float tail = 0.f;
  if constexpr (LEN > 0) {
#pragma unroll
    for (int e = (LEN / 32) * 32; e < LEN; e++) {
      const float xv = x[e], yv = y[e];
      if constexpr (KIND == 1) { const float d = xv - yv; tail = __builtin_fmaf(d, d, tail); }
      else tail = __builtin_fmaf(xv, yv, tail);
    }
  } else {
    for (; i < len; i++) {
      const float xv = x[i], yv = y[i];
      if constexpr (KIND == 1) { const float d = xv - yv; tail = __builtin_fmaf(d, d, tail); }
      else tail = __builtin_fmaf(xv, yv, tail);
    }
  }
  float s[8];
#pragma unroll
  for (int j = 0; j < 8; j++) s[j] = ((acc[j] + acc[8 + j]) + acc[16 + j]) + acc[24 + j];
  float t0 = s[0] + s[4], t1 = s[1] + s[5], t2 = s[2] + s[6], t3 = s[3] + s[7];
  t0 = t0 + tail; t1 = t1 + 0.0f; t2 = t2 + 0.0f; t3 = t3 + 0.0f;
  const float h0 = t0 + t1, h1 = t2 + t3;
  const float r = h0 + h1;
  if constexpr (KIND == 0) return 1.0f - r;
  else if constexpr (KIND == 2) return -r;
  else return r;
}

template <int KIND>
__global__ __launch_bounds__(256) void pq_lut_kernel(const float* __restrict__ cb, int m, int C, int dsub, const float* __restrict__ queries,
                                                     int mp, float* __restrict__ lut, uint32_t* __restrict__ cnt, uint32_t* __restrict__ thr,
                                                     uint32_t* __restrict__ ovf) {
  const int j = blockIdx.x, q = blockIdx.y, c = threadIdx.x;
  if (cnt && j == 0 && c == 0) { cnt[q] = 0; thr[q] = 0xffffffffu; if (q == 0) *ovf = 0; }
  float v = 0.f;
  if (j < m && c < C) v = pq_dist<KIND>(queries + ((size_t)q * m + j) * dsub, cb + ((size_t)j * C + c) * dsub, dsub);
  lut[((size_t)q * mp + j) * 256 + c] = v;
}

template <int KIND>
__global__ __launch_bounds__(256) void pq_lut16_max_kernel(const float* __restrict__ cb, int m, int C, int dsub, const float* __restrict__ queries,
                                                           int mp, int shift, uint32_t* __restrict__ qmax) {
  const int per = 256 >> shift;
  const int j = blockIdx.x * per + ((int)threadIdx.x >> shift), c = (int)threadIdx.x & ((1 << shift) - 1), q = blockIdx.y;
  float v = 0.f;
  if (j < m && c < C) v = pq_dist<KIND>(queries + ((size_t)q * m + j) * dsub, cb + ((size_t)j * C + c) * dsub, dsub);
  uint32_t b = v > 0.f ? __float_as_uint(v) : 0u;
#pragma unroll
  for (int o = 32; o >= 1; o >>= 1) { const uint32_t t = (uint32_t)__shfl_xor((int)b, o, 64); b = t > b ? t : b; }
  if ((threadIdx.x & 63) == 0 && b) atomicMax(&qmax[q], b);
}
__device__ __forceinline__ float pq_table_scale(uint32_t max_bits) {
  const float M = __uint_as_float(max_bits);
  float s = 1.0f;
  if (M == M && M < __uint_as_float(0x7f800000u)) { while (M * s > 32768.0f) s *= 0.5f; }
  return s;
}
template <int KIND>
__global__ __launch_bounds__(256) void pq_lut16_kernel(const float* __restrict__ cb, int m, int C, int dsub, const float* __restrict__ queries,
                                                       int mp, int shift, const uint32_t* __restrict__ qmax, unsigned short* __restrict__ lut) {
  const int per = 256 >> shift;
  const int j = blockIdx.x * per + ((int)threadIdx.x >> shift), c = (int)threadIdx.x & ((1 << shift) - 1), q = blockIdx.y;
  if (j >= mp) return;
  float v = 0.f;
  if (j < m && c < C) v = pq_dist<KIND>(queries + ((size_t)q * m + j) * dsub, cb + ((size_t)j * C + c) * dsub, dsub);
  v = v * pq_table_scale(qmax[q]);
  lut[(((size_t)q * mp + j) << shift) + c] = (unsigned short)f32bits_to_f16bits(__float_as_uint(v));
}
__global__ void pq_centroid_norm_max_kernel(const float* __restrict__ cb, uint32_t n_centroids, int dsub, uint32_t* __restrict__ out) {
  const uint32_t i = blockIdx.x * blockDim.x + threadIdx.x;
  float s = 0.f;
  if (i < n_centroids) for (int e = 0; e < dsub; e++) { const float x = cb[(size_t)i * dsub + e]; s = __builtin_fmaf(x, x, s); }
  if (i < n_centroids) atomicMax(out, s == s ? __float_as_uint(s) : 0x7fc00000u);
}

__device__ __forceinline__ size_t code_offset(uint64_t row, int j, int T, int PB) {
  return (((row >> 6) * (uint64_t)T + (uint64_t)(j / PB)) * 64 + (row & 63)) * PB + (j % PB);
}
template <int DS>
__global__ __launch_bounds__(256) void pq_encode_kernel(const float* __restrict__ cb, int m, int C, int dsub, const float* __restrict__ vecs,
                                                        uint64_t n, const uint32_t* __restrict__ slots, uint64_t slot_base, int lds_cb,
                                                        uint8_t* __restrict__ codes, int T, int PB) {
  extern __shared__ __attribute__((aligned(16))) float s_cb[];
  const int j = blockIdx.y;
  const float* cbj = cb + (size_t)j * C * dsub;
  if (lds_cb) {
    for (int i = threadIdx.x; i < C * dsub; i += blockDim.x) s_cb[i] = cbj[i];
    __syncthreads();
    cbj = s_cb;
  }
  const uint64_t i = (uint64_t)blockIdx.x * blockDim.x + threadIdx.x;
  if (i >= n) return;
  const float* x = vecs + (i * (uint64_t)m + j) * dsub;
  float minDist = 3.40282346638528859811704183484516925440e+38f;
  int best = 0;
  if constexpr (DS > 0) {
    float xr[DS];
#pragma unroll
    for (int e = 0; e < DS; e++) xr[e] = x[e];
    for (int c = 0; c < C; c++) {
      const float d = pq_dist<1, DS>(xr, cbj + (size_t)c * DS, DS);
      if (d < minDist) { minDist = d; best = c; }
    }
  } else {
    for (int c = 0; c < C; c++) {
      const float d = pq_dist<1>(x, cbj + (size_t)c * dsub, dsub);
      if (d < minDist) { minDist = d; best = c; }
    }
  }
  const uint64_t row = slots ? slots[i] : slot_base + i;
  codes[code_offset(row, j, T, PB)] = (uint8_t)best;
}

__global__ void pq_place_codes_kernel(const uint8_t* __restrict__ src, uint64_t n, int m, int C, const uint32_t* __restrict__ slots, uint64_t slot_base,
                                      uint8_t* __restrict__ codes, int T, int PB, uint32_t* __restrict__ bad) {
  const uint64_t t = (uint64_t)blockIdx.x * blockDim.x + threadIdx.x;
  if (t >= n * (uint64_t)m) return;
  const uint64_t i = t / m; const int j = (int)(t - i * m);
  const uint8_t c = src[t];
  if ((int)c >= C) { atomicAdd(bad, 1u); return; }
  codes[code_offset(slots ? slots[i] : slot_base + i, j, T, PB)] = c;
}
__global__ void pq_fetch_codes_kernel(const uint8_t* __restrict__ codes, int T, int PB, uint64_t first, uint64_t n, int m, uint8_t* __restrict__ out) {
  const uint64_t t = (uint64_t)blockIdx.x * blockDim.x + threadIdx.x;
  if (t >= n * (uint64_t)m) return;
  const uint64_t i = t / m; const int j = (int)(t - i * m);
  out[t] = codes[code_offset(first + i, j, T, PB)];
}
__global__ void pq_move_row_kernel(uint8_t* __restrict__ codes, int T, int PB, int mp, uint64_t dst, uint64_t src) {
  const int j = (int)(blockIdx.x * blockDim.x + threadIdx.x);
  if (j < mp) codes[code_offset(dst, j, T, PB)] = codes[code_offset(src, j, T, PB)];
}

__global__ void pq_train_init_kernel(const float* __restrict__ vecs, int m, int C, int dsub, float* __restrict__ cb) {
  const uint64_t t = (uint64_t)blockIdx.x * blockDim.x + threadIdx.x;
  if (t >= (uint64_t)m * C * dsub) return;
  const int e = (int)(t % dsub); const int c = (int)((t / dsub) % C); const int j = (int)(t / ((uint64_t)dsub * C));
  cb[t] = vecs[((size_t)c * m + j) * dsub + e];
}
// ... 707 lines not shown
    for (size_t i = 0; i < n * p->m; i++) if (codes[i] >= p->C) return fail(COLTT_E_INVALID, "pq upsert_codes: code %u >= numCentroids %u", (unsigned)codes[i], p->C);
  const bool dense_ok = !ids && p->dense && (p->n == 0 || first_id == p->dense_base + p->n);
  PqPlan pl; std::vector<size_t> keep;
  const uint32_t* d_slots = nullptr; uint64_t slot_base = p->n; size_t m_rows = n;
  const float* src_v = vecs; const uint8_t* src_c = codes;
  std::vector<float> v2; std::vector<uint8_t> c2; std::vector<uint32_t> s2;
  if (dense_ok) {
    if (p->n + n > 0xffffffffull) return fail(COLTT_E_UNSUPPORTED, "pq upsert: more than 2^32-1 rows in one store");
    COLTT_TRY(p->reserve(p->n + n));
  } else {
    COLTT_TRY(p->undense());
    COLTT_TRY(plan_upsert(p, ids, first_id, n, pl));
    COLTT_TRY(p->reserve(pl.nn));
    last_wins(pl, n, keep);
    const uint32_t* sl = pl.slots.data();
    if (!keep.empty()) {
      if (on_device) return fail(COLTT_E_UNSUPPORTED, "pq upsert_device: an id is repeated inside the batch");
      s2.reserve(keep.size());
      for (size_t i : keep) {
        s2.push_back(pl.slots[i]);
        if (vecs) v2.insert(v2.end(), vecs + i * p->dim, vecs + (i + 1) * p->dim);
        else c2.insert(c2.end(), codes + i * p->m, codes + (i + 1) * p->m);
      }
      sl = s2.data(); m_rows = s2.size(); src_v = vecs ? v2.data() : nullptr; src_c = codes ? c2.data() : nullptr;
    }
    COLTT_TRY(p->w_slots.reserve(m_rows * 4));
    COLTT_HIP(hipMemcpyAsync(p->w_slots.p, sl, m_rows * 4, hipMemcpyHostToDevice, p->stream));
    d_slots = p->w_slots.as<uint32_t>(); slot_base = 0;
  }
  if (vecs) {
    const float* d_v = src_v;
    if (!on_device) {
      COLTT_TRY(p->w_raw.reserve(m_rows * p->dim * 4));
      COLTT_HIP(hipMemcpyAsync(p->w_raw.p, src_v, m_rows * p->dim * 4, hipMemcpyHostToDevice, p->stream));
      d_v = p->w_raw.as<float>();
    }
    COLTT_TRY(launch_encode(p, p->stream, d_v, m_rows, d_slots, slot_base, p->codes.as<uint8_t>()));
  } else {
    COLTT_TRY(p->w_raw.reserve(m_rows * p->m));
    COLTT_HIP(hipMemcpyAsync(p->w_raw.p, src_c, m_rows * p->m, hipMemcpyHostToDevice, p->stream));
    COLTT_HIP(hipMemsetAsync(p->w_bad.p, 0, 4, p->stream));
    pq_place_codes_kernel<<<ceil_div(m_rows * p->m, 256), 256, 0, p->stream>>>(p->w_raw.as<uint8_t>(), m_rows, (int)p->m, (int)p->C, d_slots, slot_base,
                                                                              p->codes.as<uint8_t>(), p->T, p->PB, p->w_bad.as<uint32_t>());
    COLTT_HIP(hipGetLastError());
  }
  if (!dense_ok && !pl.new_ids.empty())
    COLTT_HIP(hipMemcpyAsync(p->ids.as<uint64_t>() + p->n, pl.new_ids.data(), pl.new_ids.size() * 8, hipMemcpyHostToDevice, p->stream));
  COLTT_HIP(hipStreamSynchronize(p->stream));
  if (dense_ok) { if (p->n == 0) p->dense_base = first_id; p->n += n; }
  else commit_upsert(p, pl);
  return COLTT_OK;
}

int coltt_pq_upsert(coltt_handle_t h, const uint64_t* ids, const float* vecs, size_t n) {
  auto p = lookup<Pq>(h);
  if (!p) return fail(COLTT_E_NOT_FOUND, "pq_upsert: unknown handle");
  if (n == 0) return COLTT_OK;
  if (!ids || !vecs) return fail(COLTT_E_INVALID, "pq_upsert: NULL input");
  WriteLock g(p->rw);
  COLTT_DEVICE(p->device);
  return pq_upsert_impl(p.get(), ids, 0, vecs, false, nullptr, n);
}

int coltt_pq_upsert_device(coltt_handle_t h, const uint64_t* ids, uint64_t first_id, const float* d_vecs, size_t n) {
  auto p = lookup<Pq>(h);
  if (!p) return fail(COLTT_E_NOT_FOUND, "pq_upsert_device: unknown handle");
  if (n == 0) return COLTT_OK;
  if (!d_vecs) return fail(COLTT_E_INVALID, "pq_upsert_device: NULL vectors");
  WriteLock g(p->rw);
  COLTT_DEVICE(p->device);
  return pq_upsert_impl(p.get(), ids, first_id, d_vecs, true, nullptr, n);
}

int coltt_pq_upsert_codes(coltt_handle_t h, const uint64_t* ids, const uint8_t* codes, size_t n) {
  auto p = lookup<Pq>(h);
  if (!p) return fail(COLTT_E_NOT_FOUND, "pq_upsert_codes: unknown handle");
  if (n == 0) return COLTT_OK;
  if (!ids || !codes) return fail(COLTT_E_INVALID, "pq_upsert_codes: NULL input");
  WriteLock g(p->rw);
  COLTT_DEVICE(p->device);
  return pq_upsert_impl(p.get(), ids, 0, nullptr, false, codes, n);
}

int coltt_pq_remove(coltt_handle_t h, const uint64_t* ids, size_t n) {
  auto p = lookup<Pq>(h);
  if (!p) return fail(COLTT_E_NOT_FOUND, "pq_remove: unknown handle");
  if (n == 0) return COLTT_OK;
  if (!ids) return fail(COLTT_E_INVALID, "pq_remove: NULL ids");
  WriteLock g(p->rw);
  COLTT_DEVICE(p->device);
  COLTT_TRY(p->undense());
  for (size_t i = 0; i < n; i++) {
    auto it = p->id2slot.find(ids[i]);
    if (it == p->id2slot.end()) continue;
    const uint32_t s = it->second; const uint64_t last = p->n - 1;
    p->id2slot.erase(it);
    if (s != last) {
      pq_move_row_kernel<<<(p->mp + 255) / 256, 256, 0, p->stream>>>(p->codes.as<uint8_t>(), p->T, p->PB, p->mp, s, last);
      const uint64_t moved = p->h_ids[last];
      p->h_ids[s] = moved; p->id2slot[moved] = s;
      COLTT_HIP(hipMemcpyAsync(p->ids.as<uint64_t>() + s, p->ids.as<uint64_t>() + last, 8, hipMemcpyDeviceToDevice, p->stream));
    }
    p->h_ids.pop_back();
    p->n--;
  }
  COLTT_HIP(hipGetLastError());
  COLTT_HIP(hipStreamSynchronize(p->stream));
  return COLTT_OK;
}

int coltt_pq_len(coltt_handle_t h, uint64_t* out) {
  auto p = lookup<Pq>(h);
  if (!p || !out) return fail(COLTT_E_NOT_FOUND, "pq_len: unknown handle");
  ReadLock g(p->rw);
  *out = p->n;
  return COLTT_OK;
}

int coltt_pq_fetch_codes(coltt_handle_t h, uint64_t first_slot, uint64_t n, uint8_t* out_codes, uint64_t* out_ids) {
  auto p = lookup<Pq>(h);
  if (!p) return fail(COLTT_E_NOT_FOUND, "pq_fetch_codes: unknown handle");
  if (n == 0) return COLTT_OK;
  ReadLock g(p->rw);
  COLTT_DEVICE(p->device);
  if (first_slot + n > p->n) return fail(COLTT_E_INVALID, "pq_fetch_codes: range outside [0,%llu)", (unsigned long long)p->n);
  if (out_codes) {
    DevBuf d_o;
    COLTT_TRY(d_o.reserve(n * p->m));
    pq_fetch_codes_kernel<<<ceil_div(n * p->m, 256), 256>>>(p->codes.as<uint8_t>(), p->T, p->PB, first_slot, n, (int)p->m, d_o.as<uint8_t>());
    COLTT_HIP(hipGetLastError());
    COLTT_HIP(hipMemcpy(out_codes, d_o.p, n * p->m, hipMemcpyDeviceToHost));
  }
  if (out_ids) for (uint64_t i = 0; i < n; i++) out_ids[i] = p->dense ? p->dense_base + first_slot + i : p->h_ids[first_slot + i];
  return COLTT_OK;
}

int coltt_pq_lut(coltt_handle_t h, const float* query, float* out_lut) {
  auto p = lookup<Pq>(h);
  if (!p) return fail(COLTT_E_NOT_FOUND, "pq_lut: unknown handle");
  if (!query || !out_lut) return fail(COLTT_E_INVALID, "pq_lut: NULL buffer");
  ReadLock g(p->rw);
  COLTT_DEVICE(p->device);
  if (!p->trained) return fail(COLTT_E_INVALID, "pq_lut: no codebooks yet");
  DevBuf d_q, d_l;
  COLTT_TRY(d_q.reserve((size_t)p->dim * 4)); COLTT_TRY(d_l.reserve((size_t)p->mp * 256 * 4));
  COLTT_HIP(hipMemcpy(d_q.p, query, (size_t)p->dim * 4, hipMemcpyHostToDevice));
  dim3 grid(p->mp, 1);
  if (p->metric == COLTT_PQ_COSINE) pq_lut_kernel<0><<<grid, 256>>>(p->cb.as<float>(), (int)p->m, (int)p->C, (int)p->dsub, d_q.as<float>(), p->mp, d_l.as<float>(), nullptr, nullptr, nullptr);
  else if (p->metric == COLTT_PQ_EUCLIDEAN) pq_lut_kernel<1><<<grid, 256>>>(p->cb.as<float>(), (int)p->m, (int)p->C, (int)p->dsub, d_q.as<float>(), p->mp, d_l.as<float>(), nullptr, nullptr, nullptr);
  else pq_lut_kernel<2><<<grid, 256>>>(p->cb.as<float>(), (int)p->m, (int)p->C, (int)p->dsub, d_q.as<float>(), p->mp, d_l.as<float>(), nullptr, nullptr, nullptr);
  COLTT_HIP(hipGetLastError());
  COLTT_HIP(hipMemcpy2D(out_lut, (size_t)p->C * 4, d_l.p, 256 * 4, (size_t)p->C * 4, p->m, hipMemcpyDeviceToHost));
  return COLTT_OK;
}

int coltt_pq_search(coltt_handle_t h, const float* queries, size_t nq, uint32_t k, uint64_t* out_ids, float* out_scores, uint32_t* out_counts) {
  auto p = lookup<Pq>(h);
  if (!p) return fail(COLTT_E_NOT_FOUND, "pq_search: unknown handle");
  if (nq && (!queries || !out_ids || !out_scores || !out_counts)) return fail(COLTT_E_INVALID, "pq_search: NULL buffer");
  ReadLock g(p->rw);
  COLTT_DEVICE(p->device);
  CtxLease<PCtx> ctx(p->pool);
  if (!ctx.c) return COLTT_E_DEVICE;
  return pq_search_common(p.get(), ctx.c, queries, false, nq, k, out_ids, out_scores, out_counts, false);
}

// ... 23 lines not shown
```

### coltt_amd/hnsw.py

```python
import ctypes as C

import numpy as np

from . import _lib as L


class HnswCfg(C.Structure):
    _fields_ = [("m", C.c_int32), ("m_max", C.c_int32), ("m_max0", C.c_int32), ("ef", C.c_int32),
                ("ef_construction", C.c_int32), ("algo", C.c_int32), ("level_multiplier", C.c_float),
                ("extend_candidates", C.c_int32), ("keep_pruned", C.c_int32)]

    @staticmethod
    def default(**kw):
        c = HnswCfg(16, -1, -1, 20, 200, 0, -1.0, 0, 1)
        for k, v in kw.items():
            setattr(c, k, v)
        return c


class HnswStats(C.Structure):
    _fields_ = [("n_dist", C.c_uint64), ("n_exp", C.c_uint64), ("n_hops", C.c_uint64), ("n_visit_resets", C.c_uint64)]


FILTER_AUTO, FILTER_WALK, FILTER_EXACT = 0, 1, 2
# ... 401 lines not shown
    def SearchFiltered(self, queries, k, flt, ef=0, mode=FILTER_AUTO, with_stats=False):
        q = np.ascontiguousarray(queries, np.float32).reshape(-1, self.dim)
        nq = q.shape[0]
        ids = np.zeros((nq, k), np.uint64); sc = np.zeros((nq, k), np.float32); cnt = np.zeros(nq, np.uint32)
        st = HnswFilterStats()
        L.check(L.lib().coltt_hnsw_search_filtered(self.h, flt.h, L.vp(q), C.c_size_t(nq), C.c_uint32(k), C.c_uint32(ef), C.c_int(int(mode)),
                                                   L.vp(ids), L.vp(sc), L.vp(cnt), C.byref(st)))
        if with_stats:
            return ids, sc, cnt, {"n_dist": st.n_dist, "n_exp": st.n_exp, "n_hops": st.n_hops, "n_visit_resets": st.n_visit_resets,
                                  "ef_walk": st.ef_walk, "path": st.path, "n_exact_rows": st.n_exact_rows}
        return ids, sc, cnt

    def SearchFilteredBatch(self, queries, k, filters, ef=0, mode=FILTER_AUTO, with_stats=False):
        q = np.ascontiguousarray(queries, np.float32).reshape(-1, self.dim)
        nq = q.shape[0]
        if len(filters) != nq:
            raise ValueError(f"SearchFilteredBatch: {len(filters)} filters for {nq} queries")
        fh = np.array([0 if f.h is None else f.h.value for f in filters], np.uint64)
        ids = np.zeros((nq, k), np.uint64); sc = np.zeros((nq, k), np.float32); cnt = np.zeros(nq, np.uint32)
        paths = np.zeros(nq, np.int32)
        st = HnswFilterStats()
        L.check(L.lib().coltt_hnsw_search_filtered_batch(self.h, L.vp(fh), L.vp(q), C.c_size_t(nq), C.c_uint32(k), C.c_uint32(ef),
                                                         C.c_int(int(mode)), L.vp(ids), L.vp(sc), L.vp(cnt), L.vp(paths), C.byref(st)))
        if with_stats:
            return ids, sc, cnt, paths, {"n_dist": st.n_dist, "n_exp": st.n_exp, "n_hops": st.n_hops, "n_visit_resets": st.n_visit_resets,
                                         "ef_walk": st.ef_walk, "path": st.path, "n_exact_rows": st.n_exact_rows}
        return ids, sc, cnt, paths

    def SearchDevice(self, d_q, nq, k, d_ids, d_scores, d_counts, ef=0):
        st = HnswStats()
        L.check(L.lib().coltt_hnsw_search_device(self.h, C.c_void_p(d_q), C.c_size_t(nq), C.c_uint32(k), C.c_uint32(ef),
                                                 C.c_void_p(d_ids), C.c_void_p(d_scores), C.c_void_p(d_counts), C.byref(st)))
        return {"n_dist": st.n_dist, "n_exp": st.n_exp, "n_hops": st.n_hops, "n_visit_resets": st.n_visit_resets}

    def Export(self):
        ns, nr, ne, ent = C.c_uint64(0), C.c_uint64(0), C.c_uint64(0), C.c_int32(0)
        L.check(L.lib().coltt_hnsw_export(self.h, C.byref(ns), C.byref(nr), C.byref(ne), None, None, None, None, None, None, C.byref(ent)))
        ids = np.empty(ns.value, np.uint64); lv = np.empty(ns.value, np.int32); dl = np.empty(ns.value, np.uint8)
        off = np.empty(nr.value + 1, np.int64); nb = np.empty(ne.value, np.int32); nd = np.empty(ne.value, np.float32)
        L.check(L.lib().coltt_hnsw_export(self.h, C.byref(ns), C.byref(nr), C.byref(ne), L.vp(ids), L.vp(lv), L.vp(dl), L.vp(off),
                                          L.vp(nb), L.vp(nd), C.byref(ent)))
        return {"ids": ids, "levels": lv, "deleted": dl, "row_offsets": off, "nbr": nb, "nbr_dist": nd, "entry": ent.value}

    def Commit(self, header=True):
        n = C.c_uint64(0)
        L.check(L.lib().coltt_hnsw_commit(self.h, int(header), None, None, C.c_uint64(0), None, C.c_uint64(0), C.byref(n)))
        buf = np.empty(n.value, np.uint8)
        L.check(L.lib().coltt_hnsw_commit(self.h, int(header), None, None, C.c_uint64(0), L.vp(buf), C.c_uint64(n.value), C.byref(n)))
        return buf.tobytes()

    def Load(self, data, header=True):
        b = np.frombuffer(data, np.uint8)
        n = C.c_uint64(0)
        L.check(L.lib().coltt_hnsw_load(self.h, int(header), L.vp(b), C.c_uint64(len(b)), C.byref(n), None, None, None, C.c_uint64(0)))
        L.check(L.lib().coltt_hnsw_get_cfg(self.h, C.byref(self.cfg)))
        return n.value

    def ExportRaw(self):
        ns, nu, ent, el = C.c_uint64(0), C.c_uint64(0), C.c_int32(0), C.c_int32(0)
        L.check(L.lib().coltt_hnsw_export_raw(self.h, C.byref(ns), C.byref(nu), C.byref(ent), C.byref(el), None, None, None))
        adj0 = np.empty((ns.value, self.cfg.m_max0), np.uint32); uo = np.empty(ns.value, np.uint32)
        adjU = np.empty((max(nu.value, 1), self.cfg.m_max), np.uint32)
        L.check(L.lib().coltt_hnsw_export_raw(self.h, C.byref(ns), C.byref(nu), C.byref(ent), C.byref(el), L.vp(adj0), L.vp(uo), L.vp(adjU)))
        return {"adj0": adj0, "upper_off": uo, "adjU": adjU, "entry": ent.value, "entry_level": el.value, "n": ns.value}

    def FetchRows(self, first=0, n=None, out=None):
        ns = C.c_uint64(0)
        L.check(L.lib().coltt_hnsw_export_raw(self.h, C.byref(ns), None, None, None, None, None, None))
        n = ns.value - first if n is None else n
        dt = {L.Q_NONE: np.float32, L.Q_F8: np.uint8}.get(self.quantization, np.uint16)
        if out is None:
            out = np.empty((n, self.dim), dt)
        L.check(L.lib().coltt_hnsw_fetch_rows(self.h, C.c_uint64(first), C.c_uint64(n), L.vp(out)))
        return out

    def Reserve(self, n_slots, n_upper_rows=0):
        L.check(L.lib().coltt_hnsw_reserve(self.h, C.c_uint64(int(n_slots)), C.c_uint64(int(n_upper_rows))))

    def Rows8(self):
        a, f = C.c_uint64(0), C.c_int32(0)
        L.check(L.lib().coltt_hnsw_rows8_searches(self.h, C.byref(a), C.byref(f)))
        return a.value, bool(f.value)

    def RowFilterStats(self):
        r, e, s, n, f = C.c_uint64(0), C.c_uint64(0), C.c_uint64(0), C.c_uint64(0), C.c_int32(0)
        L.check(L.lib().coltt_hnsw_row_filter_stats(self.h, C.byref(r), C.byref(e), C.byref(s), C.byref(n), C.byref(f)))
        us, ur, uf, un = C.c_uint64(0), C.c_uint64(0), C.c_uint64(0), C.c_uint64(0)
        L.check(L.lib().coltt_hnsw_row_filter_stats_ex(self.h, C.byref(us), C.byref(ur), C.byref(uf), C.byref(un)))
        return {"rejected": r.value, "f32_rows": e.value, "shadow_rows": s.value, "launches": n.value, "shadow": bool(f.value),
                "shadow_bits": tuple(b for b in (8, 16) if f.value & b),
                "upper_shadow_rows": us.value, "upper_rejected": ur.value, "upper_f32_rows": uf.value, "upper_launches": un.value}

    def VisitedStats(self):
        k, w, g = C.c_int32(0), C.c_uint32(0), C.c_uint32(0)
        n, s, v = C.c_uint64(0), C.c_uint64(0), C.c_uint64(0)
        L.check(L.lib().coltt_hnsw_visited_stats(self.h, C.byref(k), C.byref(w), C.byref(g), C.byref(n), C.byref(s), C.byref(v)))
        return {"kind": k.value, "waves_per_cu": w.value, "grid": g.value, "launches16": n.value, "stash_max": s.value, "visited_max": v.value}

    def PlanFacts(self):
        f = PlanFactsC()
        L.check(L.lib().coltt_hnsw_search_plan_facts(self.h, C.byref(f)))
        return f

    def SearchPlan(self, nq, k, ef=0, force=0):
        return search_plan_host(self.PlanFacts(), nq, k, ef or self.cfg.ef, force)

    def FetchShadow8(self, first=0, n=None):
        ns = C.c_uint64(0)
        L.check(L.lib().coltt_hnsw_export_raw(self.h, C.byref(ns), None, None, None, None, None, None))
        n = ns.value - first if n is None else n
        codes = np.empty((n, self.dim), np.int8); meta = np.empty((n, 2), np.float32); adj = np.empty((n, self.cfg.m_max0, 2), np.float32)
        L.check(L.lib().coltt_hnsw_fetch_shadow8(self.h, C.c_uint64(first), C.c_uint64(n), L.vp(codes), L.vp(meta), L.vp(adj)))
        return codes, meta, adj

    def RowFilterProbe(self, queries, slots, lower_bound, bits=8, nt=0, full_at_pop=1, sums=False):
        q = np.ascontiguousarray(queries, np.float32).reshape(-1, self.dim)
        nq = q.shape[0]
        s = np.ascontiguousarray(slots, np.uint32).reshape(nq, 32)
        lb = np.ascontiguousarray(np.broadcast_to(np.asarray(lower_bound, np.float32), (nq,)))
        r = np.zeros((nq, 32), np.float32); qn = np.zeros(nq, np.float32); rn = np.zeros((nq, 32), np.float32); cnt = np.zeros((nq, 3), np.uint32)
        if bits in ("8i", 80):
            isum = np.zeros((nq, 32), np.int64); qte = np.zeros((nq, 2), np.float32)
            L.check(L.lib().coltt_hnsw_row_filter_probe_ex(self.h, L.vp(q), C.c_size_t(nq), L.vp(s), L.vp(lb), C.c_int(80), C.c_int(int(nt)),
                                                           C.c_int(int(full_at_pop)), L.vp(r), L.vp(qn), L.vp(rn), L.vp(cnt), L.vp(isum), L.vp(qte)))
            return (r, qn, rn, cnt, isum, qte) if sums else (r, qn, rn, cnt)
        if sums:
            raise ValueError("RowFilterProbe: only the \"8i\" kind forms integer sums")
        L.check(L.lib().coltt_hnsw_row_filter_probe(self.h, L.vp(q), C.c_size_t(nq), L.vp(s), L.vp(lb), C.c_int(int(bits)), C.c_int(int(nt)),
                                                    C.c_int(int(full_at_pop)), L.vp(r), L.vp(qn), L.vp(rn), L.vp(cnt)))
        return r, qn, rn, cnt

    def PqAttach(self, pq):
        L.check(L.lib().coltt_hnsw_pq_attach(self.h, pq.h))

    def PqInfo(self):
        m, c, mt, n = C.c_uint32(0), C.c_uint32(0), C.c_int32(0), C.c_uint64(0)
        L.check(L.lib().coltt_hnsw_pq_info(self.h, C.byref(m), C.byref(c), C.byref(mt), C.byref(n)))
        return {"m": m.value, "C": c.value, "metric": mt.value, "coded": n.value}

    def PqCodes(self, first=0, n=None):
        info = self.PqInfo()
        n = info["coded"] - first if n is None else n
        out = np.empty((n, info["m"]), np.uint8)
        L.check(L.lib().coltt_hnsw_pq_fetch_codes(self.h, C.c_uint64(first), C.c_uint64(n), L.vp(out)))
        return out

    def PqNbrStats(self):
        b, p, r, s = C.c_uint64(0), C.c_uint64(0), C.c_uint64(0), C.c_int32(0)
        L.check(L.lib().coltt_hnsw_pq_nbr_stats(self.h, C.byref(b), C.byref(p), C.byref(r), C.byref(s)))
        return {"builds": b.value, "patches": p.value, "patched_rows": r.value, "state": s.value}

    def PqFetchNbr(self, first=0, n=None):
        ns = C.c_uint64(0)
        L.check(L.lib().coltt_hnsw_export_raw(self.h, C.byref(ns), None, None, None, None, None, None))
        n = ns.value - first if n is None else n
        out = np.empty((n, self.cfg.m_max0, (self.PqInfo()["m"] + 15) & ~15), np.uint8)
        L.check(L.lib().coltt_hnsw_pq_fetch_nbr(self.h, C.c_uint64(first), C.c_uint64(n), L.vp(out)))
        return out

    def PqSearch(self, queries, k, ef=0, rerank=0, with_stats=False):
        q = np.ascontiguousarray(queries, np.float32).reshape(-1, self.dim)
        nq = q.shape[0]
        ids = np.zeros((nq, k), np.uint64); sc = np.zeros((nq, k), np.float32); cnt = np.zeros(nq, np.uint32)
        st = HnswStats(); nx = C.c_uint64(0)
        L.check(L.lib().coltt_hnsw_pq_search(self.h, L.vp(q), C.c_size_t(nq), C.c_uint32(k), C.c_uint32(ef), C.c_uint32(rerank), L.vp(ids), L.vp(sc),
                                             L.vp(cnt), C.byref(st), C.byref(nx)))
# ... 43 lines not shown
```

### include/coltt_gpu.h

```cpp
#ifndef COLTT_GPU_H
#define COLTT_GPU_H
#include <stddef.h>
#include <stdint.h>
#ifdef __cplusplus
extern "C" {
#endif

typedef uint64_t coltt_handle_t;

enum { COLTT_OK = 0, COLTT_E_INVALID = -1, COLTT_E_EXISTS = -2, COLTT_E_NOT_FOUND = -3,
       COLTT_E_UNSUPPORTED = -4, COLTT_E_DEVICE = -5, COLTT_E_NOMEM = -6 };

enum { COLTT_COSINE = 0, COLTT_EUCLIDEAN = 1 };
enum { COLTT_MANHATTAN = 2 };
enum { COLTT_Q_NONE = 0, COLTT_Q_F16 = 1, COLTT_Q_F8 = 2, COLTT_Q_BF16 = 3 };
enum { COLTT_SELECT_REFERENCE = 0, COLTT_SELECT_NEAREST = 1 };
enum { COLTT_MODE_EXACT = 0, COLTT_MODE_MFMA = 1 };

int coltt_init(int device);
int coltt_device_count(void);
const char* coltt_last_error(void);
const char* coltt_version(void);
int coltt_policy_reload(void);

// ... 95 lines not shown
#define COLTT_FILTER_AUTO 0
#define COLTT_FILTER_WALK 1
#define COLTT_FILTER_EXACT 2
typedef struct coltt_hnsw_filter_stats {
  uint64_t n_dist, n_exp, n_hops, n_visit_resets;
  uint32_t ef_walk;
  int32_t path;
  uint64_t n_exact_rows;
} coltt_hnsw_filter_stats;
int coltt_hnsw_filter_create(coltt_handle_t hnsw, const uint64_t* ids, size_t n, uint64_t* out_allowed, coltt_handle_t* out);
int coltt_hnsw_filter_destroy(coltt_handle_t filter);
int coltt_hnsw_search_filtered(coltt_handle_t hnsw, coltt_handle_t filter, const float* queries, size_t nq, uint32_t k,
                               uint32_t ef_override, int mode, uint64_t* out_ids, float* out_scores, uint32_t* out_counts,
                               coltt_hnsw_filter_stats* stats);
int coltt_hnsw_search_filtered_batch(coltt_handle_t hnsw, const coltt_handle_t* filters , const float* queries, size_t nq,
                                     uint32_t k, uint32_t ef_override, int mode, uint64_t* out_ids, float* out_scores,
                                     uint32_t* out_counts, int32_t* out_paths , coltt_hnsw_filter_stats* stats);

int coltt_hnsw_pq_search_filtered(coltt_handle_t hnsw, coltt_handle_t filter, const float* queries, size_t nq, uint32_t k, uint32_t ef_override_or_0,
                                  uint32_t rerank, int mode , uint64_t* out_ids, float* out_scores, uint32_t* out_counts,
                                  coltt_hnsw_filter_stats* stats);
int coltt_hnsw_pq_search_filtered_batch(coltt_handle_t hnsw, const coltt_handle_t* filters , const float* queries, size_t nq,
                                        uint32_t k, uint32_t ef_override_or_0, uint32_t rerank, int mode ,
                                        uint64_t* out_ids, float* out_scores, uint32_t* out_counts,
                                        int32_t* out_paths , coltt_hnsw_filter_stats* stats);

#define COLTT_FOP_AND    (-1)
#define COLTT_FOP_OR     (-2)
#define COLTT_FOP_ANDNOT (-3)
#define COLTT_FOP_NOT    (-4)
#define COLTT_FOP_ALL    (-5)
int coltt_hnsw_filter_eval(coltt_handle_t hnsw, const int32_t* prog, size_t n_prog, const coltt_handle_t* leaves, size_t n_leaves,
                           uint64_t* out_allowed, coltt_handle_t* out);
int coltt_hnsw_filter_eval_batch(coltt_handle_t hnsw, const int32_t* progs, const uint64_t* prog_off , size_t n_out,
                                 const coltt_handle_t* leaves, size_t n_leaves, uint64_t* out_allowed ,
                                 coltt_handle_t* out );
int coltt_hnsw_filter_ids(coltt_handle_t filter, uint64_t* out_ids, uint64_t cap, uint64_t* out_n);
int coltt_hnsw_filter_info(coltt_handle_t filter, coltt_handle_t* out_index, uint64_t* out_allowed, uint64_t* out_slots);
int coltt_hnsw_filter_prog_check_host(const int32_t* prog, size_t n_prog, size_t n_leaves, uint32_t* out_depth);

#define COLTT_ATTR_I64 0
#define COLTT_ATTR_F64 1
#define COLTT_CMP_EQ 0
#define COLTT_CMP_NE 1
#define COLTT_CMP_GT 2
#define COLTT_CMP_GE 3
#define COLTT_CMP_LT 4
#define COLTT_CMP_LE 5
#define COLTT_CMP_SET 6
typedef struct coltt_attr_pred {
  coltt_handle_t column;
  int32_t op;
  int32_t reserved;
  union { int64_t i64; double f64; } value;
} coltt_attr_pred;
int coltt_hnsw_attr_create(coltt_handle_t hnsw, int type, coltt_handle_t* out);
int coltt_hnsw_attr_destroy(coltt_handle_t column);
int coltt_hnsw_attr_set(coltt_handle_t column, const uint64_t* ids, const void* values , size_t n,
                        uint64_t* out_applied);
int coltt_hnsw_attr_get(coltt_handle_t column, const uint64_t* ids, size_t n, void* out_values, uint8_t* out_set);
int coltt_hnsw_attr_info(coltt_handle_t column, coltt_handle_t* out_index, int32_t* out_type, uint64_t* out_slots, uint64_t* out_set);
int coltt_hnsw_filter_eval_attr(coltt_handle_t hnsw, const int32_t* prog, size_t n_prog, const coltt_handle_t* leaves, size_t n_leaves,
                                const coltt_attr_pred* preds, size_t n_preds, uint64_t* out_allowed, coltt_handle_t* out);
int coltt_hnsw_filter_eval_attr_batch(coltt_handle_t hnsw, const int32_t* progs, const uint64_t* prog_off , size_t n_out,
                                      const coltt_handle_t* leaves, size_t n_leaves, const coltt_attr_pred* preds, size_t n_preds,
                                      uint64_t* out_allowed , coltt_handle_t* out );
int coltt_attr_cmp_host(int type, int op, const void* operand, const void* value, int is_set);

int coltt_hnsw_reserve(coltt_handle_t h, uint64_t n_slots, uint64_t n_upper_rows);

typedef struct coltt_hnsw_compact_stats {
  uint64_t slots_before, slots_after;
  uint64_t upper_rows_before, upper_rows_after;
  uint64_t edges_dropped;
  uint64_t rows_moved;
  uint64_t bytes_moved;
  float    ms;
} coltt_hnsw_compact_stats;
int coltt_hnsw_compact(coltt_handle_t h, uint64_t stage_bytes_or_0, uint32_t* out_new_of_old , uint64_t cap_map,
                       coltt_hnsw_compact_stats* stats );
int coltt_hnsw_compact_map_host(const uint32_t* del_bits, uint64_t n_slots, const int32_t* levels, uint32_t* out_new_of_old,
                                uint32_t* out_new_upper_off, uint64_t* out_live, uint64_t* out_upper_rows);
int coltt_hnsw_rows8_searches(coltt_handle_t h, uint64_t* out_launches, int32_t* out_has_copy);
int coltt_hnsw_row_filter_stats(coltt_handle_t h, uint64_t* out_rejected, uint64_t* out_f32_rows, uint64_t* out_shadow_rows, uint64_t* out_launches, int32_t* out_has_shadow);
int coltt_hnsw_row_filter_stats_ex(coltt_handle_t h, uint64_t* out_upper_shadow_rows, uint64_t* out_upper_rejected, uint64_t* out_upper_f32_rows, uint64_t* out_upper_launches);
int coltt_hnsw_visited_stats(coltt_handle_t h, int32_t* out_kind, uint32_t* out_waves_per_cu, uint32_t* out_grid, uint64_t* out_launches16, uint64_t* out_stash_max, uint64_t* out_visited_max);
typedef struct coltt_hnsw_plan_facts {
  uint32_t dim; int32_t metric, quant;
  uint32_t m_max0;
  uint64_t stride;
  uint64_t slots;
  int32_t r8;
  int32_t shadow8, shadow16;
  int32_t vis_ready;
  uint32_t vis_regions;
} coltt_hnsw_plan_facts;
enum { COLTT_PLAN_LATENCY = 0, COLTT_PLAN_WALK2 = 1, COLTT_PLAN_ONE_WAVE = 2 };
typedef struct coltt_hnsw_search_plan {
  int32_t family;
  uint32_t ef, ef_pad;
  uint32_t hcap;
  uint64_t lds;
  int32_t vis_kind;
  int32_t w2;
  uint32_t bloom_words;
  int32_t r8;
  int32_t ev8;
  int32_t nt;
  int32_t filter;
  uint32_t upper;
  uint32_t v16_bits, v16_limit;
  uint32_t per_cu, grid;
  int32_t rows8_launch;
  int32_t lat_seq, lat_helpers;
} coltt_hnsw_search_plan;
int coltt_hnsw_search_plan_host(const coltt_hnsw_plan_facts* facts, size_t nq, uint32_t k, uint32_t ef_override, int force, coltt_hnsw_search_plan* out);
int coltt_hnsw_search_plan_facts(coltt_handle_t h, coltt_hnsw_plan_facts* out_facts);
int coltt_hnsw_fetch_shadow8(coltt_handle_t h, uint64_t first_slot, uint64_t n, int8_t* out_codes, float* out_meta, float* out_adj_meta);
int coltt_hnsw_row_filter_probe(coltt_handle_t h, const float* queries, size_t nq, const uint32_t* slots, const float* lower_bound, int bits, int nt,
                                int full_at_pop, float* out_r, float* out_qnorm, float* out_rnorm, uint32_t* out_counts);
int coltt_hnsw_row_filter_probe_ex(coltt_handle_t h, const float* queries, size_t nq, const uint32_t* slots, const float* lower_bound, int bits, int nt,
                                   int full_at_pop, float* out_r, float* out_qnorm, float* out_rnorm, uint32_t* out_counts, int64_t* out_isum, float* out_qte);
int coltt_hnsw_export(coltt_handle_t h, uint64_t* n_slots, uint64_t* n_rows, uint64_t* n_edges, uint64_t* ids,
                      int32_t* levels, uint8_t* deleted, int64_t* row_offsets, int32_t* nbr, float* nbr_dist,
                      int32_t* entry_slot);
int coltt_hnsw_commit(coltt_handle_t h, int header, const uint8_t* const* meta_blobs, const uint32_t* meta_lens, uint64_t n_meta,
                      uint8_t* out, uint64_t cap, uint64_t* out_len);
int coltt_hnsw_entry_level(coltt_handle_t h, int32_t* out_level);
int coltt_hnsw_load(coltt_handle_t h, int header, const uint8_t* buf, uint64_t len, uint64_t* out_n, uint64_t* out_ids,
                    uint64_t* out_meta_off, uint32_t* out_meta_len, uint64_t cap_n);
int coltt_hnsw_export_raw(coltt_handle_t h, uint64_t* n_slots, uint64_t* n_upper_rows, int32_t* entry_slot,
                          int32_t* entry_level, uint32_t* adj0, uint32_t* upper_off, uint32_t* adjU);
int coltt_hnsw_get(coltt_handle_t h, uint64_t id, void* out_row, int32_t* out_level);
int coltt_hnsw_fetch_rows(coltt_handle_t h, uint64_t first_slot, uint64_t n, void* out_rows);
int coltt_last_kernel_ms(coltt_handle_t h, float* out_ms);
int coltt_last_kernel_ms_flat(coltt_handle_t h, float* out_ms);

enum { COLTT_GROUP_FLAT = 0, COLTT_GROUP_HNSW = 1 };
enum { COLTT_LAYOUT_SHARD = 0, COLTT_LAYOUT_REPLICA = 1 };
enum { COLTT_EXCHANGE_AUTO = 0, COLTT_EXCHANGE_RCCL = 1, COLTT_EXCHANGE_HOST = 2,
       COLTT_EXCHANGE_SHM = 3  };
#define COLTT_UNIQUE_ID_BYTES 128
typedef struct coltt_group_opts {
  int32_t kind;
  int32_t layout;
  int32_t exchange;
  int32_t world_size;
  int32_t rank_base;
  const uint8_t* unique_id;
} coltt_group_opts;
int coltt_group_unique_id(uint8_t* out );
int coltt_shm_open(const uint8_t* unique_id, int world, int n_local, int rank_base, uint64_t bytes_per_rank, coltt_handle_t* out);
int coltt_shm_allgather(coltt_handle_t h, const void* local, uint64_t bytes, void* out);
int coltt_shm_close(coltt_handle_t h);
int coltt_group_create(const int* devices, int n_devices, uint32_t dim, int metric, int quant, const coltt_hnsw_cfg* cfg,
                       const coltt_group_opts* opts, coltt_handle_t* out);
int coltt_group_destroy(coltt_handle_t h);
int coltt_group_info(coltt_handle_t h, int32_t* n_local, int32_t* world, int32_t* exchange_in_use, int32_t* rank_base);
int coltt_group_member(coltt_handle_t h, int i, coltt_handle_t* out);
int coltt_group_shard_of(coltt_handle_t h, uint64_t id, int32_t* out_shard);
int coltt_group_upsert(coltt_handle_t h, const uint64_t* ids, const float* vecs, size_t n, uint64_t* out_kept);
int coltt_group_insert(coltt_handle_t h, const uint64_t* ids, const float* vecs, const int32_t* levels, size_t n, uint32_t batch,
                       uint64_t* out_kept);
int coltt_group_remove(coltt_handle_t h, const uint64_t* ids, size_t n);
int coltt_group_len(coltt_handle_t h, uint64_t* out);
int coltt_group_search(coltt_handle_t h, const float* queries, size_t nq, uint32_t k, int select, int mode, uint32_t ef_override,
                       uint64_t* out_ids, float* out_scores, uint32_t* out_counts);
int coltt_group_search_device(coltt_handle_t h, const float* const* d_queries_per_member, size_t nq, uint32_t k, int select, int mode,
                              uint32_t ef_override, uint64_t* out_ids, float* out_scores, uint32_t* out_counts);
int coltt_group_search_begin(coltt_handle_t h, const float* queries, const float* const* d_queries_per_member, size_t nq, uint32_t k,
                             int select, int mode, uint32_t ef_override, uint64_t* out_ids, float* out_scores, uint32_t* out_counts,
                             uint64_t* out_ticket);
int coltt_group_search_end(coltt_handle_t h, uint64_t ticket);
int coltt_group_timing(coltt_handle_t h, double* out4);
int coltt_group_merge_host(const void* recs, int world, size_t nq, uint32_t k, int nearest, uint64_t* out_ids, float* out_scores,
                           uint32_t* out_counts);
int coltt_group_first_failed_rank_host(const void* recs, int world, size_t per, uint32_t* out_status);
uint64_t coltt_shard_vertex_host(uint64_t id, uint64_t shard_count);

enum { COLTT_PQ_COSINE = 0 , COLTT_PQ_EUCLIDEAN = 1 ,
       COLTT_PQ_DOT = 2  };
int coltt_pq_create(uint32_t dim, int metric, uint32_t num_subvectors, uint32_t num_centroids, coltt_handle_t* out);
int coltt_pq_destroy(coltt_handle_t h);
int coltt_pq_set_codebooks(coltt_handle_t h, const float* codebooks);
int coltt_pq_get_codebooks(coltt_handle_t h, float* out_codebooks);
int coltt_pq_train(coltt_handle_t h, const float* vecs, size_t n, uint32_t iterations);
int coltt_pq_encode(coltt_handle_t h, const float* vecs, size_t n, uint8_t* out_codes);
int coltt_pq_upsert(coltt_handle_t h, const uint64_t* ids, const float* vecs, size_t n);
int coltt_pq_upsert_device(coltt_handle_t h, const uint64_t* ids, uint64_t first_id, const float* d_vecs, size_t n);
int coltt_pq_upsert_codes(coltt_handle_t h, const uint64_t* ids, const uint8_t* codes, size_t n);
int coltt_pq_remove(coltt_handle_t h, const uint64_t* ids, size_t n);
int coltt_pq_len(coltt_handle_t h, uint64_t* out);
int coltt_pq_fetch_codes(coltt_handle_t h, uint64_t first_slot, uint64_t n, uint8_t* out_codes, uint64_t* out_ids);
int coltt_pq_lut(coltt_handle_t h, const float* query, float* out_lut);
int coltt_pq_search(coltt_handle_t h, const float* queries, size_t nq, uint32_t k, uint64_t* out_ids, float* out_scores,
                    uint32_t* out_counts);
int coltt_pq_search_device(coltt_handle_t h, const float* d_queries, size_t nq, uint32_t k, uint64_t* d_out_ids, float* d_out_scores,
                           uint32_t* d_out_counts);
int coltt_pq_last_kernel_ms(coltt_handle_t h, float* out_search_ms, float* out_scan_ms, uint64_t* out_scan_rows);


int coltt_hnsw_pq_attach(coltt_handle_t hnsw, coltt_handle_t pq);
int coltt_hnsw_pq_info(coltt_handle_t hnsw, uint32_t* out_num_subvectors, uint32_t* out_num_centroids, int32_t* out_pq_metric, uint64_t* out_coded_slots);
int coltt_hnsw_pq_fetch_codes(coltt_handle_t hnsw, uint64_t first_slot, uint64_t n, uint8_t* out_codes);
int coltt_hnsw_pq_nbr_stats(coltt_handle_t hnsw, uint64_t* out_builds, uint64_t* out_patches,
                            uint64_t* out_patched_rows, int32_t* out_state);
int coltt_hnsw_pq_fetch_nbr(coltt_handle_t hnsw, uint64_t first_slot, uint64_t n, uint8_t* out_blocks);
int coltt_hnsw_pq_search(coltt_handle_t hnsw, const float* queries, size_t nq, uint32_t k, uint32_t ef_override_or_0, uint32_t rerank,
                         uint64_t* out_ids, float* out_scores, uint32_t* out_counts, coltt_hnsw_stats* stats, uint64_t* out_n_exact);
int coltt_hnsw_pq_search_device(coltt_handle_t hnsw, const float* d_queries, size_t nq, uint32_t k, uint32_t ef_override_or_0, uint32_t rerank,
                                uint64_t* d_out_ids, float* d_out_scores, uint32_t* d_out_counts, coltt_hnsw_stats* stats, uint64_t* out_n_exact);

#ifdef __cplusplus
}
#endif
#endif
```

Baseline: 1.148 million.

## Build PQ lookup tables inside the HNSW walk kernel instead of a separate launch

Adds a path where each wave of the PQ HNSW walk kernel computes its own query's f16 distance table from the codebook and the query into LDS, rather than a separate pq_lut16_batch kernel writing tables to global memory that the walk then copies in. It is on by default for 32-entry rows with 12-float subvectors, and for 256-entry rows with 24-float subvectors when the batch has at least 8 queries. This removes a kernel launch, the global table buffer and its round trip, and lets all queries go in a single group. In exchange each wave does the table arithmetic itself, including a second pass when rescaling is needed, which adds compute and codebook reads per query and may delay the start of the walk.

```diff
diff --git a/coltt_amd/_lib.py b/coltt_amd/_lib.py
--- a/coltt_amd/_lib.py
+++ b/coltt_amd/_lib.py
@@ -12,7 +12,7 @@
 _lib = None
 _env_seen = None
 _KNOBS = ("COLTT_FLAT_ONE", "COLTT_FLAT_IDS_CHUNK", "COLTT_STAGING", "COLTT_EV8", "COLTT_ROWS8", "COLTT_F8_MFMA", "COLTT_VISG", "COLTT_WALK2", "COLTT_WALK2_LDS", "COLTT_BLOOM_KB",
-          "COLTT_WAVES_PER_CU", "COLTT_ROWS_NT", "COLTT_ROWS_NT_MIN_MB", "COLTT_ROW_FILTER", "COLTT_ROW_FILTER_BITS", "COLTT_ROW_FILTER_UPPER", "COLTT_DESCENT_NT", "COLTT_ROW_SHADOW", "COLTT_ROW_SHADOW_BITS", "COLTT_VIS16", "COLTT_VIS16_BUCKET_BITS", "COLTT_PQ_WAVES", "COLTT_PQ_NBR", "COLTT_PQ_NBR_PATCH", "COLTT_LAT_SEQ", "COLTT_LAT_HELPERS", "COLTT_LAT_MAX_NQ", "COLTT_MW_MAX_NQ", "COLTT_VISG_BUDGET_MB")
+          "COLTT_WAVES_PER_CU", "COLTT_ROWS_NT", "COLTT_ROWS_NT_MIN_MB", "COLTT_ROW_FILTER", "COLTT_ROW_FILTER_BITS", "COLTT_ROW_FILTER_UPPER", "COLTT_DESCENT_NT", "COLTT_ROW_SHADOW", "COLTT_ROW_SHADOW_BITS", "COLTT_VIS16", "COLTT_VIS16_BUCKET_BITS", "COLTT_PQ_WAVES", "COLTT_PQ_NBR", "COLTT_PQ_NBR_PATCH", "COLTT_PQ_TABLE", "COLTT_LAT_SEQ", "COLTT_LAT_HELPERS", "COLTT_LAT_MAX_NQ", "COLTT_MW_MAX_NQ", "COLTT_VISG_BUDGET_MB")
 
 
 class ColttError(RuntimeError):
diff --git a/coltt_amd/csrc/common.hip b/coltt_amd/csrc/common.hip
--- a/coltt_amd/csrc/common.hip
+++ b/coltt_amd/csrc/common.hip
@@ -92,6 +92,7 @@
   v = num("COLTT_PQ_WAVES", set); p.pq_waves = set ? (int)std::max<long long>(1, std::min<long long>(16, v)) : 0;
   p.pq_nbr = !off("COLTT_PQ_NBR");
   p.pq_nbr_patch = !off("COLTT_PQ_NBR_PATCH");
+  { const char* e = getenv("COLTT_PQ_TABLE"); p.pq_table = (!e || !*e) ? -1 : (!strcmp(e, "walk") ? 1 : (!strcmp(e, "launch") ? 0 : -1)); }
   { const char* e = getenv("COLTT_LAT_SEQ"); p.lat_seq = e && *e == '1'; }
   v = num("COLTT_LAT_HELPERS", set); p.lat_helpers = set ? (int)std::max<long long>(0, std::min<long long>(3, v)) : 0;
   v = num("COLTT_LAT_MAX_NQ", set); if (!set) v = num("COLTT_MW_MAX_NQ", set);
diff --git a/coltt_amd/csrc/common.hpp b/coltt_amd/csrc/common.hpp
--- a/coltt_amd/csrc/common.hpp
+++ b/coltt_amd/csrc/common.hpp
@@ -113,6 +113,7 @@
   int vis16_bucket_bits = 0;
   int pq_waves = 0;
   bool pq_nbr = true;
+  int pq_table = -1;
   bool pq_nbr_patch = true;
   bool lat_seq = false;
   int lat_helpers = 0;
diff --git a/coltt_amd/csrc/hnsw.hip b/coltt_amd/csrc/hnsw.hip
--- a/coltt_amd/csrc/hnsw.hip
+++ b/coltt_amd/csrc/hnsw.hip
@@ -984,11 +984,16 @@
 namespace hnsw {
 int launch_pq_walk(Hnsw* x, HCtx* c, const PqGeom& sg, bool nbr, uint32_t grid, uint32_t region_base, const unsigned short* lut, uint32_t nq, uint32_t k,
                    uint32_t rerank, uint32_t* counter, uint32_t* surv, uint32_t* surv_cnt, unsigned long long* stats, const FilterView* fv, uint32_t fcap,
-                   const PqFiltQuery* pd) {
+                   const PqFiltQuery* pd, const float* table_q) {
   const uint32_t sh = pq_lut_shift(x);
+  if (table_q && (fv || pd || !(sh == 4 || sh == 5 || sh == 8))) return fail(COLTT_E_INVALID, "hnsw_pq_search: no walk instance builds its own table for this call (filtered, or rows of %u entries)", 1u << sh);
+  const PqShape& ps = x->pq_shape;
+  if (table_q && (ps.m > 128 || ps.C > 256 || ps.dsub >= (1u << 14))) return fail(COLTT_E_INVALID, "hnsw_pq_search: quantiser shape %u x %u x %u", ps.m, ps.C, ps.dsub);
+  const PqTableSrc ts{table_q ? x->pq_cb.as<float>() : nullptr, table_q,
+                      PqTableSrc::pack(ps.m, ps.C, ps.dsub, ps.metric == COLTT_PQ_COSINE ? 0u : ps.metric == COLTT_PQ_EUCLIDEAN ? 1u : 2u)};
   const uint32_t np = x->pq_row >> 4;
   typedef void (*pq_kern_t)(GraphView, int32_t, int32_t, const unsigned short*, const uint8_t*, const uint8_t*, uint32_t, uint32_t, uint32_t, uint32_t, uint32_t, uint32_t, uint32_t, uint32_t,
-                            uint32_t*, uint32_t*, uint32_t*, unsigned long long*, uint8_t*, size_t, uint32_t*, FilterView, uint32_t);
+                            uint32_t*, uint32_t*, uint32_t*, unsigned long long*, uint8_t*, size_t, uint32_t*, FilterView, uint32_t, PqTableSrc);
   pq_kern_t kern;
 #define COLTT_PQKF(LS, NP, F, P) (sg.variant == 0 ? (pq_kern_t)hnsw_pq_search_kernel<0, VIS_LDS, LS, NP, false, F, P> : nbr ? (pq_kern_t)hnsw_pq_search_kernel<2, VIS_HBM, LS, NP, true, F, P> : (pq_kern_t)hnsw_pq_search_kernel<2, VIS_HBM, LS, NP, false, F, P>)
 #define COLTT_PQK(LS, NP) (pd ? COLTT_PQKF(LS, NP, true, true) : fv ? COLTT_PQKF(LS, NP, true, false) : COLTT_PQKF(LS, NP, false, false))
@@ -1006,8 +1011,9 @@
   kern<<<grid, 64, sg.lds, c->stream>>>(x->view(), x->entry, x->entry_level, lut, x->pq_codes.as<uint8_t>(), nbr ? x->pq_nbr.as<uint8_t>() : nullptr, x->pq_row, sh, nq, k, sg.ef, sg.ef_pad, rerank,
                                         sg.vis_words, counter, surv, surv_cnt, stats, x->w_visg.as<uint8_t>() + (size_t)region_base * x->vis_stride,
                                         (size_t)x->vis_stride, x->w_vepoch.as<uint32_t>() + region_base,
-                                        pd ? FilterView{reinterpret_cast<const uint32_t*>(pd), 0u} : fv ? *fv : FilterView{nullptr, 0u}, fcap);
+                                        pd ? FilterView{reinterpret_cast<const uint32_t*>(pd), 0u} : fv ? *fv : FilterView{nullptr, 0u}, fcap, ts);
   COLTT_HIP(hipGetLastError());
+  if (table_q) x->pq_table_walks.fetch_add(1);
   return COLTT_OK;
 }
 }
@@ -1132,8 +1138,11 @@
   if (sg.variant != 0) COLTT_TRY(ensure_pq_nbr(x, c->stream, &nbr));
   const uint32_t lsh = pq_lut_shift(x);
   const size_t lut_q = ((size_t)x->pq_row << lsh) * 2;
-  const size_t group = std::max<size_t>(1, std::min<size_t>({nq, (256ull << 20) / lut_q, (256ull << 20) / ((size_t)sg.ef_pad * 12), (size_t)32768}));
-  COLTT_TRY(c->w_pack.reserve(group * lut_q + group * 4));
+  const int tmode = policy().pq_table;
+  const bool table_can = !fv && (lsh == 4 || lsh == 5 || lsh == 8);
+  const bool table_walk = table_can && (tmode == 1 || (tmode < 0 && pq_walk_table_default(lsh, x->pq_shape.dsub, nq)));
+  const size_t group = std::max<size_t>(1, std::min<size_t>({nq, table_walk ? nq : (256ull << 20) / lut_q, (256ull << 20) / ((size_t)sg.ef_pad * 12), (size_t)32768}));
+  if (!table_walk) COLTT_TRY(c->w_pack.reserve(group * lut_q + group * 4));
   COLTT_TRY(c->w_surv.reserve(group * sg.ef_pad * 4)); COLTT_TRY(c->w_scnt.reserve(group * 4)); COLTT_TRY(c->w_keys.reserve(group * sg.ef_pad * 8));
   COLTT_TRY(c->w_misc.reserve(256));
   uint8_t* misc = c->w_misc.as<uint8_t>();
@@ -1143,11 +1152,12 @@
   COLTT_HIP(hipEventRecord(c->ev0, c->stream));
   for (size_t q0 = 0; q0 < nq; q0 += group) {
     const size_t gn = std::min(group, nq - q0);
-    COLTT_TRY(pq_lut16_batch(c->stream, x->pq_cb.as<float>(), x->pq_shape, c->w_qeff.as<float>() + q0 * x->dim, gn, x->pq_row, lsh,
-                             reinterpret_cast<uint32_t*>(c->w_pack.as<uint8_t>() + group * lut_q), c->w_pack.as<unsigned short>()));
+    if (!table_walk)
+      COLTT_TRY(pq_lut16_batch(c->stream, x->pq_cb.as<float>(), x->pq_shape, c->w_qeff.as<float>() + q0 * x->dim, gn, x->pq_row, lsh,
+                               reinterpret_cast<uint32_t*>(c->w_pack.as<uint8_t>() + group * lut_q), c->w_pack.as<unsigned short>()));
     if (q0) COLTT_HIP(hipMemsetAsync(counter, 0, 4, c->stream));
-    COLTT_TRY(launch_pq_walk(x, c, sg, nbr, (uint32_t)std::min<size_t>(grid, gn), lease.base, c->w_pack.as<unsigned short>(), (uint32_t)gn, k, rerank, counter, c->w_surv.as<uint32_t>(),
-                             c->w_scnt.as<uint32_t>(), d_stats, fv, fcap));
+    COLTT_TRY(launch_pq_walk(x, c, sg, nbr, (uint32_t)std::min<size_t>(grid, gn), lease.base, table_walk ? nullptr : c->w_pack.as<unsigned short>(), (uint32_t)gn, k, rerank, counter,
+                             c->w_surv.as<uint32_t>(), c->w_scnt.as<uint32_t>(), d_stats, fv, fcap, nullptr, table_walk ? c->w_qeff.as<float>() + q0 * x->dim : nullptr));
     COLTT_TRY(launch_pq_rerank(x, c, sg, (uint32_t)q0, (uint32_t)gn, k, c->w_surv.as<uint32_t>(), c->w_scnt.as<uint32_t>(), c->w_keys.as<unsigned long long>(), d_oi, d_os, d_oc));
   }
   COLTT_HIP(hipEventRecord(c->ev1, c->stream));
@@ -2348,6 +2358,13 @@
   return pq_search_common(x.get(), ctx.c, d_queries, true, nq, k, ef_override, rerank, d_out_ids, d_out_scores, d_out_counts, stats, out_n_exact);
 }
 
+int coltt_hnsw_pq_table_walks(coltt_handle_t h, uint64_t* out_launches) {
+  auto x = lookup<Hnsw>(h);
+  if (!x) return fail(COLTT_E_NOT_FOUND, "hnsw_pq_table_walks: unknown handle");
+  if (out_launches) *out_launches = x->pq_table_walks.load();
+  return COLTT_OK;
+}
+
 int coltt_hnsw_rows8_searches(coltt_handle_t h, uint64_t* out_launches, int32_t* out_has_copy) {
   auto x = lookup<Hnsw>(h);
   if (!x) return fail(COLTT_E_NOT_FOUND, "hnsw_rows8_searches: unknown handle");
diff --git a/coltt_amd/csrc/hnsw_index.hpp b/coltt_amd/csrc/hnsw_index.hpp
--- a/coltt_amd/csrc/hnsw_index.hpp
+++ b/coltt_amd/csrc/hnsw_index.hpp
@@ -63,6 +63,7 @@
   bool pq_nbr_built = false;
   DevBuf pq_dirty;
   std::atomic<uint64_t> pq_nbr_builds{0}, pq_nbr_patches{0}, pq_nbr_patched_rows{0};
+  std::atomic<uint64_t> pq_table_walks{0};
   bool dense = true; uint64_t dense_base = 0;
   std::unordered_map<uint64_t, uint32_t> id2slot;
   std::vector<uint64_t> h_ids;
@@ -178,7 +179,7 @@
 int pq_walk_geom(Hnsw* x, uint32_t ef, bool force_hbm, uint32_t fcap, PqGeom& sg);
 int launch_pq_walk(Hnsw* x, HCtx* c, const PqGeom& sg, bool nbr, uint32_t grid, uint32_t region_base, const unsigned short* lut, uint32_t nq, uint32_t k,
                    uint32_t rerank, uint32_t* counter, uint32_t* surv, uint32_t* surv_cnt, unsigned long long* stats, const FilterView* fv = nullptr, uint32_t fcap = 0,
-                   const PqFiltQuery* pd = nullptr);
+                   const PqFiltQuery* pd = nullptr, const float* table_q = nullptr);
 int launch_pq_rerank(Hnsw* x, HCtx* c, const PqGeom& sg, uint32_t q0, uint32_t nq, uint32_t k, const uint32_t* surv, const uint32_t* surv_cnt,
                      unsigned long long* keys, uint64_t* oi, float* os, uint32_t* oc, const PqFiltQuery* pd = nullptr, const float* pd_qe = nullptr,
                      const float* pd_qn = nullptr);
diff --git a/coltt_amd/csrc/hnsw_kernels.hpp b/coltt_amd/csrc/hnsw_kernels.hpp
--- a/coltt_amd/csrc/hnsw_kernels.hpp
+++ b/coltt_amd/csrc/hnsw_kernels.hpp
@@ -476,7 +476,7 @@
                                                             uint32_t ef, uint32_t ef_pad, uint32_t rerank, uint32_t vis_words,
                                                             uint32_t* __restrict__ counter, uint32_t* __restrict__ surv, uint32_t* __restrict__ surv_cnt,
                                                             unsigned long long* __restrict__ stats, uint8_t* __restrict__ visg,
-                                                            size_t vis_stride, uint32_t* __restrict__ vis_epoch, FilterView fv, uint32_t fcap) {
+                                                            size_t vis_stride, uint32_t* __restrict__ vis_epoch, FilterView fv, uint32_t fcap, PqTableSrc ts) {
   extern __shared__ __attribute__((aligned(16))) uint8_t smem[];
   const int lane = threadIdx.x;
   WaveCtx w;
@@ -527,7 +527,18 @@
     w.t_last = __builtin_amdgcn_s_memtime();
 #endif
     wave_sync();
-    {
+    bool built = false;
+    if constexpr (!FILTER && LS != 0) {
+      if (ts.cb != nullptr) {
+        PqTableSrc t = ts;
+        asm volatile("" : "+s"(t.cb), "+s"(t.q), "+s"(t.shape));
+        if (t.kind() == 0) pq_walk_table_len<0>(lut, t, qi, row_bytes, lut_shift, lane);
+        else if (t.kind() == 1) pq_walk_table_len<1>(lut, t, qi, row_bytes, lut_shift, lane);
+        else pq_walk_table_len<2>(lut, t, qi, row_bytes, lut_shift, lane);
+        built = true;
+      }
+    }
+    if (!built) {
       const u32x4v* src = reinterpret_cast<const u32x4v*>(lut_g + ((size_t)qi * row_bytes << lut_shift));
       u32x4v* dst = reinterpret_cast<u32x4v*>(lut);
       const uint32_t psh = lut_shift - 3;
diff --git a/coltt_amd/csrc/hnsw_pq.hpp b/coltt_amd/csrc/hnsw_pq.hpp
--- a/coltt_amd/csrc/hnsw_pq.hpp
+++ b/coltt_amd/csrc/hnsw_pq.hpp
@@ -1,10 +1,77 @@
 #pragma once
 #include "hnsw_walk2.hpp"
+#include "pq_dist.hpp"
 
 namespace coltt {
 namespace dev {
 
 __host__ __device__ __forceinline__ constexpr uint32_t pq_walk_table_rows(uint32_t pieces) { return 2u * ((pieces + 1u) / 2u) * 16u; }
+
+template <int KIND, int LEN>
+__device__ __forceinline__ void pq_walk_table(unsigned short* lut, const PqTableSrc& ts, uint32_t qi, uint32_t row_bytes, uint32_t shift, int lane) {
+  const uint32_t total = row_bytes << shift;
+  const uint32_t js = 16u * (((row_bytes >> 4) + 1u) >> 1), cmask = (1u << shift) - 1u;
+  const uint32_t dsub = LEN > 0 ? (uint32_t)LEN : ts.dsub(), tm = ts.m(), tC = ts.C();
+  const float* const q = ts.q + (size_t)qi * tm * dsub;
+  constexpr int U = LEN == 0 ? 1 : (LEN <= 12 ? 4 : 2);
+  float scale = 1.0f;
+  for (int pass = 0; pass < 2; pass++) {
+    uint32_t mx = 0;
+    for (uint32_t i0 = (uint32_t)lane; i0 < total; i0 += 64u * U) {
+      float v[U];
+      if constexpr (LEN > 0) {
+        static_assert(LEN % 4 == 0, "16-byte loads");
+        f32x4 xa[U][LEN / 4], ya[U][LEN / 4];
+#pragma unroll
+        for (int u = 0; u < U; u++) {
+          const uint32_t i = i0 + 64u * u, j = i >> shift, c = i & cmask;
+          const bool live = j < tm && c < tC;
+          const uint32_t jj = live ? j : 0u, cc = live ? c : 0u;
+          const f32x4* const xp = reinterpret_cast<const f32x4*>(q + (size_t)jj * LEN);
+          const f32x4* const yp = reinterpret_cast<const f32x4*>(ts.cb + ((size_t)jj * tC + cc) * LEN);
+#pragma unroll
+          for (int e = 0; e < LEN / 4; e++) { xa[u][e] = xp[e]; ya[u][e] = yp[e]; }
+        }
+#pragma unroll
+        for (int u = 0; u < U; u++) {
+          float xr[LEN], yr[LEN];
+#pragma unroll
+          for (int e = 0; e < LEN; e++) { xr[e] = xa[u][e >> 2][e & 3]; yr[e] = ya[u][e >> 2][e & 3]; }
+          v[u] = pq_dist<KIND, LEN>(xr, yr, LEN);
+        }
+      } else {
+        const uint32_t j = i0 >> shift, c = i0 & cmask;
+        const bool live = j < tm && c < tC;
+        const uint32_t jj = live ? j : 0u, cc = live ? c : 0u;
+        v[0] = pq_dist<KIND>(q + (size_t)jj * dsub, ts.cb + ((size_t)jj * tC + cc) * dsub, (int)dsub);
+      }
+#pragma unroll
+      for (int u = 0; u < U; u++) {
+        const uint32_t i = i0 + 64u * u, j = i >> shift, c = i & cmask;
+        const float e = (j < tm && c < tC) ? v[u] : 0.f;
+        const uint32_t b = e > 0.f ? __float_as_uint(e) : 0u;
+        mx = b > mx ? b : mx;
+        const uint32_t r = j < js ? 2u * j : 2u * (j - js) + 1u;
+        lut[(r << shift) + c] = (unsigned short)f32bits_to_f16bits(__float_as_uint(e * scale));
+      }
+    }
+    if (pass == 1) break;
+#pragma unroll
+    for (int o = 32; o >= 1; o >>= 1) { const uint32_t t = (uint32_t)__shfl_xor((int)mx, o, 64); mx = t > mx ? t : mx; }
+    scale = pq_table_scale(mx);
+    if (scale == 1.0f) break;
+  }
+}
+template <int KIND>
+__device__ __forceinline__ void pq_walk_table_len(unsigned short* lut, const PqTableSrc& ts, uint32_t qi, uint32_t row_bytes, uint32_t shift, int lane) {
+  if (ts.dsub() == 12) pq_walk_table<KIND, 12>(lut, ts, qi, row_bytes, shift, lane);
+  else if (ts.dsub() == 24) pq_walk_table<KIND, 24>(lut, ts, qi, row_bytes, shift, lane);
+  else pq_walk_table<KIND, 0>(lut, ts, qi, row_bytes, shift, lane);
+}
+__host__ __device__ __forceinline__ constexpr bool pq_walk_table_default(uint32_t shift, uint32_t dsub, size_t nq) {
+  return (shift == 5 && dsub == 12) || (shift == 8 && dsub == 24 && nq >= 8);
+}
+
 template <int LS = 0, int NP = 0, bool NBR = false> struct AdcEval {
   const uint8_t* codes; uint32_t row_bytes;
   const unsigned short* lut;
diff --git a/coltt_amd/csrc/pq.hip b/coltt_amd/csrc/pq.hip
--- a/coltt_amd/csrc/pq.hip
+++ b/coltt_amd/csrc/pq.hip
@@ -4,6 +4,7 @@
 
 #include "common.hpp"
 #include "exact.hpp"
+#include "pq_dist.hpp"
 #include "select.hpp"
 
 using namespace coltt;
@@ -14,52 +15,6 @@
 typedef float f32x2 __attribute__((ext_vector_type(2)));
 constexpr int PQ_LDS_MAX = 152 * 1024;
 
-template <int KIND, int LEN = 0>
-__device__ __forceinline__ float pq_dist(const float* __restrict__ x, const float* __restrict__ y, int len_rt) {
-  const int len = LEN > 0 ? LEN : len_rt;
-  float acc[32];
-#pragma unroll
-  for (int u = 0; u < 32; u++) acc[u] = 0.f;
-#define PQ_BLOCK_(I_)                                                                                   \
-  _Pragma("unroll") for (int u = 0; u < 32; u++) {                                                      \
-    const float xv = x[(I_) + u], yv = y[(I_) + u];                                                     \
-    if constexpr (KIND == 1) { const float d = xv - yv; acc[u] = __builtin_fmaf(d, d, acc[u]); }        \
-    else acc[u] = __builtin_fmaf(xv, yv, acc[u]);                                                       \
-  }
-  int i = 0;
-  if constexpr (LEN > 0) {
-#pragma unroll
-    for (int b = 0; b < LEN / 32; b++) { PQ_BLOCK_(b * 32) }
-  } else {
-    for (; len - i >= 32; i += 32) { PQ_BLOCK_(i) }
-  }
-#undef PQ_BLOCK_
-  float tail = 0.f;
-  if constexpr (LEN > 0) {
-#pragma unroll
-    for (int e = (LEN / 32) * 32; e < LEN; e++) {
-      const float xv = x[e], yv = y[e];
-      if constexpr (KIND == 1) { const float d = xv - yv; tail = __builtin_fmaf(d, d, tail); }
-      else tail = __builtin_fmaf(xv, yv, tail);
-    }
-  } else {
-    for (; i < len; i++) {
-      const float xv = x[i], yv = y[i];
-      if constexpr (KIND == 1) { const float d = xv - yv; tail = __builtin_fmaf(d, d, tail); }
-      else tail = __builtin_fmaf(xv, yv, tail);
-    }
-  }
-  float s[8];
-#pragma unroll
-  for (int j = 0; j < 8; j++) s[j] = ((acc[j] + acc[8 + j]) + acc[16 + j]) + acc[24 + j];
-  float t0 = s[0] + s[4], t1 = s[1] + s[5], t2 = s[2] + s[6], t3 = s[3] + s[7];
-  t0 = t0 + tail; t1 = t1 + 0.0f; t2 = t2 + 0.0f; t3 = t3 + 0.0f;
-  const float h0 = t0 + t1, h1 = t2 + t3;
-  const float r = h0 + h1;
-  if constexpr (KIND == 0) return 1.0f - r;
-  else if constexpr (KIND == 2) return -r;
-  else return r;
-}
 
 template <int KIND>
 __global__ __launch_bounds__(256) void pq_lut_kernel(const float* __restrict__ cb, int m, int C, int dsub, const float* __restrict__ queries,
@@ -83,12 +38,6 @@
 #pragma unroll
   for (int o = 32; o >= 1; o >>= 1) { const uint32_t t = (uint32_t)__shfl_xor((int)b, o, 64); b = t > b ? t : b; }
   if ((threadIdx.x & 63) == 0 && b) atomicMax(&qmax[q], b);
-}
-__device__ __forceinline__ float pq_table_scale(uint32_t max_bits) {
-  const float M = __uint_as_float(max_bits);
-  float s = 1.0f;
-  if (M == M && M < __uint_as_float(0x7f800000u)) { while (M * s > 32768.0f) s *= 0.5f; }
-  return s;
 }
 template <int KIND>
 __global__ __launch_bounds__(256) void pq_lut16_kernel(const float* __restrict__ cb, int m, int C, int dsub, const float* __restrict__ queries,
@@ -962,6 +911,22 @@
   return pq_upsert_impl(p.get(), ids, 0, nullptr, false, codes, n);
 }
 
+int coltt_pq_dist_host(int metric, const float* x, const float* y, uint32_t len, size_t n, uint32_t compiled_len, float* out, float* out_scale) {
+  if (!x || !y || !out) return fail(COLTT_E_INVALID, "pq_dist_host: NULL x, y or out");
+  if (metric != COLTT_PQ_COSINE && metric != COLTT_PQ_EUCLIDEAN && metric != COLTT_PQ_DOT) return fail(COLTT_E_INVALID, "pq_dist_host: unknown metric %d", metric);
+  if (compiled_len != 0 && (compiled_len != len || (len != 12 && len != 24))) return fail(COLTT_E_INVALID, "pq_dist_host: no compile-time form for length %u (asked: %u)", len, compiled_len);
+  for (size_t i = 0; i < n; i++) {
+    const float* a = x + i * len; const float* b = y + i * len;
+    float v;
+#define COLTT_PD(K) (compiled_len == 12 ? pq_dist<K, 12>(a, b, 12) : compiled_len == 24 ? pq_dist<K, 24>(a, b, 24) : pq_dist<K>(a, b, (int)len))
+    if (metric == COLTT_PQ_COSINE) v = COLTT_PD(0); else if (metric == COLTT_PQ_EUCLIDEAN) v = COLTT_PD(1); else v = COLTT_PD(2);
+#undef COLTT_PD
+    out[i] = v;
+    if (out_scale) { uint32_t bits = 0; if (v > 0.f) std::memcpy(&bits, &v, 4); out_scale[i] = pq_table_scale(bits); }
+  }
+  return COLTT_OK;
+}
+
 int coltt_pq_remove(coltt_handle_t h, const uint64_t* ids, size_t n) {
   auto p = lookup<Pq>(h);
   if (!p) return fail(COLTT_E_NOT_FOUND, "pq_remove: unknown handle");
diff --git a/coltt_amd/csrc/pq_dist.hpp b/coltt_amd/csrc/pq_dist.hpp
--- /dev/null
+++ b/coltt_amd/csrc/pq_dist.hpp
@@ -0,0 +1,72 @@
+#pragma once
+#include <hip/hip_runtime.h>
+#include <stdint.h>
+
+namespace coltt {
+namespace dev {
+
+template <int KIND, int LEN = 0>
+__host__ __device__ __forceinline__ float pq_dist(const float* __restrict__ x, const float* __restrict__ y, int len_rt) {
+  const int len = LEN > 0 ? LEN : len_rt;
+  float acc[32];
+#pragma unroll
+  for (int u = 0; u < 32; u++) acc[u] = 0.f;
+#define PQ_BLOCK_(I_)                                                                                   \
+  _Pragma("unroll") for (int u = 0; u < 32; u++) {                                                      \
+    const float xv = x[(I_) + u], yv = y[(I_) + u];                                                     \
+    if constexpr (KIND == 1) { const float d = xv - yv; acc[u] = __builtin_fmaf(d, d, acc[u]); }        \
+    else acc[u] = __builtin_fmaf(xv, yv, acc[u]);                                                       \
+  }
+  int i = 0;
+  if constexpr (LEN > 0) {
+#pragma unroll
+    for (int b = 0; b < LEN / 32; b++) { PQ_BLOCK_(b * 32) }
+  } else {
+    for (; len - i >= 32; i += 32) { PQ_BLOCK_(i) }
+  }
+#undef PQ_BLOCK_
+  float tail = 0.f;
+  if constexpr (LEN > 0) {
+#pragma unroll
+    for (int e = (LEN / 32) * 32; e < LEN; e++) {
+      const float xv = x[e], yv = y[e];
+      if constexpr (KIND == 1) { const float d = xv - yv; tail = __builtin_fmaf(d, d, tail); }
+      else tail = __builtin_fmaf(xv, yv, tail);
+    }
+  } else {
+    for (; i < len; i++) {
+      const float xv = x[i], yv = y[i];
+      if constexpr (KIND == 1) { const float d = xv - yv; tail = __builtin_fmaf(d, d, tail); }
+      else tail = __builtin_fmaf(xv, yv, tail);
+    }
+  }
+  float s[8];
+#pragma unroll
+  for (int j = 0; j < 8; j++) s[j] = ((acc[j] + acc[8 + j]) + acc[16 + j]) + acc[24 + j];
+  float t0 = s[0] + s[4], t1 = s[1] + s[5], t2 = s[2] + s[6], t3 = s[3] + s[7];
+  t0 = t0 + tail; t1 = t1 + 0.0f; t2 = t2 + 0.0f; t3 = t3 + 0.0f;
+  const float h0 = t0 + t1, h1 = t2 + t3;
+  const float r = h0 + h1;
+  if constexpr (KIND == 0) return 1.0f - r;
+  else if constexpr (KIND == 2) return -r;
+  else return r;
+}
+
+__host__ __device__ __forceinline__ float pq_table_scale(uint32_t max_bits) {
+  const float M = __builtin_bit_cast(float, max_bits);
+  float s = 1.0f;
+  if (M == M && M < __builtin_bit_cast(float, 0x7f800000u)) { while (M * s > 32768.0f) s *= 0.5f; }
+  return s;
+}
+
+struct PqTableSrc {
+  const float* cb; const float* q; uint32_t shape;
+  static __host__ __device__ __forceinline__ uint32_t pack(uint32_t m, uint32_t C, uint32_t dsub, uint32_t kind) { return m | ((C - 1u) << 8) | (kind << 16) | (dsub << 18); }
+  __host__ __device__ __forceinline__ uint32_t m() const { return shape & 0xffu; }
+  __host__ __device__ __forceinline__ uint32_t C() const { return ((shape >> 8) & 0xffu) + 1u; }
+  __host__ __device__ __forceinline__ uint32_t kind() const { return (shape >> 16) & 3u; }
+  __host__ __device__ __forceinline__ uint32_t dsub() const { return shape >> 18; }
+};
+
+}
+}
diff --git a/coltt_amd/hnsw.py b/coltt_amd/hnsw.py
--- a/coltt_amd/hnsw.py
+++ b/coltt_amd/hnsw.py
@@ -507,6 +507,11 @@
         L.check(L.lib().coltt_hnsw_rows8_searches(self.h, C.byref(a), C.byref(f)))
         return a.value, bool(f.value)
 
+    def PqTableWalks(self):
+        a = C.c_uint64(0)
+        L.check(L.lib().coltt_hnsw_pq_table_walks(self.h, C.byref(a)))
+        return a.value
+
     def RowFilterStats(self):
         r, e, s, n, f = C.c_uint64(0), C.c_uint64(0), C.c_uint64(0), C.c_uint64(0), C.c_int32(0)
         L.check(L.lib().coltt_hnsw_row_filter_stats(self.h, C.byref(r), C.byref(e), C.byref(s), C.byref(n), C.byref(f)))
diff --git a/include/coltt_gpu.h b/include/coltt_gpu.h
--- a/include/coltt_gpu.h
+++ b/include/coltt_gpu.h
@@ -201,6 +201,7 @@
 int coltt_hnsw_compact_map_host(const uint32_t* del_bits, uint64_t n_slots, const int32_t* levels, uint32_t* out_new_of_old,
                                 uint32_t* out_new_upper_off, uint64_t* out_live, uint64_t* out_upper_rows);
 int coltt_hnsw_rows8_searches(coltt_handle_t h, uint64_t* out_launches, int32_t* out_has_copy);
+int coltt_hnsw_pq_table_walks(coltt_handle_t h, uint64_t* out_launches);
 int coltt_hnsw_row_filter_stats(coltt_handle_t h, uint64_t* out_rejected, uint64_t* out_f32_rows, uint64_t* out_shadow_rows, uint64_t* out_launches, int32_t* out_has_shadow);
 int coltt_hnsw_row_filter_stats_ex(coltt_handle_t h, uint64_t* out_upper_shadow_rows, uint64_t* out_upper_rejected, uint64_t* out_upper_f32_rows, uint64_t* out_upper_launches);
 int coltt_hnsw_visited_stats(coltt_handle_t h, int32_t* out_kind, uint32_t* out_waves_per_cu, uint32_t* out_grid, uint64_t* out_launches16, uint64_t* out_stash_max, uint64_t* out_visited_max);
@@ -312,6 +313,7 @@
 int coltt_pq_len(coltt_handle_t h, uint64_t* out);
 int coltt_pq_fetch_codes(coltt_handle_t h, uint64_t first_slot, uint64_t n, uint8_t* out_codes, uint64_t* out_ids);
 int coltt_pq_lut(coltt_handle_t h, const float* query, float* out_lut);
+int coltt_pq_dist_host(int metric, const float* x, const float* y, uint32_t len, size_t n, uint32_t compiled_len, float* out, float* out_scale);
 int coltt_pq_search(coltt_handle_t h, const float* queries, size_t nq, uint32_t k, uint64_t* out_ids, float* out_scores,
                     uint32_t* out_counts);
 int coltt_pq_search_device(coltt_handle_t h, const float* d_queries, size_t nq, uint32_t k, uint64_t* d_out_ids, float* d_out_scores,
```

Result: slower. 1.123 million (-2.2%).
